# JoeyT1994/TensorNetworkQuantumSimulator.jl

Measured on AMD Instinct MI355X. Metric: two-site gates/sec at fixed chi (LxL TFIM Trotter layer), higher is better.
Workload: dtype c64 (ComplexF32; Gram/eigen steps in f64; the chi = 32 plane products as exact bf16 x 3 splits with f32 accumulation, TNQS_NO_BF16X3=1 for f32 matrix instructions)

## Files before the change

### include/tnqs_debug.h

```cpp
#ifndef TNQS_DEBUG_H
#define TNQS_DEBUG_H
#include <stdint.h>
#include "tnqs.h"
#ifdef __cplusplus
extern "C" {
#endif
int tnqs_dbg_jacobi(int dtype, int m, int n, void* A_inout, void* V_out, int* sweeps_out);
int tnqs_dbg_theta_svd_pre(int m, int n, int nq, void* A_inout, const void* Q, void* V_out, int* sweeps_out, int copies, int reps, double* ms_out, double* phase_us_out ,
                           int cap );
int tnqs_dbg_time_jacobi_f32(int m, int n, const void* A, int copies, int reps, double* ms_out, int* sweeps_out);
int tnqs_dbg_chol(int n, const void* G, void* L_out, void* W_out, int* fail_out, double tau);
int tnqs_dbg_fiber_gemm(int dtype, int D, int PA, int K, int PB, int Do, int No, const void* in, const void* X, void* out,
                        double* norm2_out, int use_mfma);
int tnqs_dbg_gram(int dtype, int D, int PA, int K, int PB, const void* X, const void* Y, void* out, int acc64, int use_mfma);
int tnqs_dbg_gram_fused(int PA, int K, int PB, const void* X, const void* Y, const void* M, void* out);
int tnqs_dbg_gauge_gram(int z, const int* chi, int bleg, const void* X, const void* M, void* out);
int tnqs_dbg_pair(int C0, int NMID, int NHI, const void* in, const void* Mx, const void* My, void* out);
int tnqs_dbg_pair_legs(int d, int z, const int* chi, int lx, int ly, const void* in, const void* Mx, const void* My, void* out);
int tnqs_dbg_pair_gram(int d, int z, const int* chi, int lx, int ly, const void* X, const void* Y, const void* M, void* out);
int tnqs_dbg_pair_gram2(int d, int z, const int* chi, int lx, int ly, const void* X, const void* Y, const void* Mx, const void* My, void* out_y, void* out_x);
int tnqs_dbg_bench_plane(int which, int nsites, int lx, int ly, int reps, double* ms);
#define TNQS_DBG_ROUTE_X3 1
#define TNQS_DBG_ROUTE_F32 2
#define TNQS_DBG_ROUTE_F64 3
#define TNQS_DBG_ROUTE_F64_SHARED 4
#define TNQS_DBG_ROUTE_HALF_LINES 5
#define TNQS_DBG_ROUTE_WHOLE_LINES 6
#define TNQS_DBG_ROUTE_SMALL_SCALAR 7
#define TNQS_DBG_ROUTE_SMALL_MFMA16 8
int tnqs_dbg_rowgemm(int D, int K, int nitems, const int* PA, const int* PB, const int* No, const void* in, const void* X, void* out, double* norm2_out,
                     int tpw, int* route_out);
int tnqs_dbg_gram_mfma(int nitems, const int* shape, const void* X, const void* Y, void* out, int nchunks, int* route_out);
int tnqs_dbg_pair16(int d, int nitems, const int* z, const int* chi, const int* lx, const int* ly, const void* in, const void* M, void* out, int spw, int* route_out);
int tnqs_dbg_pair_gram2x16(int d, int nitems, const int* z, const int* chi, const int* lx, const int* ly, const int* both, const void* X, const void* Y, const void* M,
                           void* out_y, void* out_x, int spw);
int tnqs_dbg_pair32(int d, int nitems, const int* z, const int* chi, const int* lx, const int* ly, const void* in, const void* M, void* out, int spw, int guard,
                    int* route_out, int* spw_out, int* wg_begin_out, int* nwg_out, int* total_wgs_out);
int tnqs_dbg_pair_gram32(int d, int nitems, const int* z, const int* chi, const int* lx, const int* ly, int form, const void* X, const void* Y, const void* M,
                         void* out_y, void* out_x, int spw, int guard, int* route_out, int* spw_out, int* wg_begin_out, int* nwg_out, int* total_wgs_out);
int tnqs_dbg_svd_tall(int nitems, const int* m, const int* n, void* A, int* chol_fail, int* polished, int* sweeps);
int tnqs_dbg_small_site(int nitems, const int* d, const int* z, const int* chi, const int* jo, const void* psi, const void* M, const int* present, int form,
                        const void* old_msg, const int* has_old, int normalize, void* out, void* new_msg, double* diff_out, int* route_out);
int tnqs_dbg_msg_finalize(int dtype, int nitems, const int* chi, const int* nchunks, const void* partials, const void* old_msg, const int* has_old, int normalize,
                          void* new_msg, double* diff_out);
int tnqs_dbg_default_sequence(tnqs_handle h, int* src, int* dst, int cap, int* n_out);
int tnqs_dbg_default_sequence_graph(int nv, int ne, const int32_t* esrc, const int32_t* edst, int* src, int* dst, int* level, int cap, int* n_out);
int tnqs_dbg_gate_schedule(int nv, int ne, const int32_t* esrc, const int32_t* edst, int ngates, const int32_t* nverts, const int32_t* verts, int update_cache,
                           int* step_of_gate, int* step_is_bp, int cap, int* nsteps_out);
int tnqs_dbg_fiber_plan(int use, int dtype, int use_mfma, int use_chi64, int nitems, const int* shape, int* launches_out, int cap, int* nlaunches_out, int* items_out);
int tnqs_dbg_loop_cgemm(int dtype, int opB, int nitems, const int* m, const int* n, const int* k, const void* A, const void* B, void* C, int guard);
int tnqs_dbg_loop_antiproject(int dtype, int nitems, const int* nr, const int* nc, void* T_inout, const void* f, const void* b);
int tnqs_dbg_loop_trace(int dtype, int nitems, const int* p, const int* q, const void* X, const void* Y, double* out_re_im);
int tnqs_dbg_loop_branch_gram(int dtype, int nitems, const int* dims, const int* order, const int* k, const void* A, const void* B, void* C, int guard);
int tnqs_dbg_msg_rescale(int dtype, int nitems, const int* chi, const void* me, const void* mer, const int* present, void* me_out, void* mer_out, int guard);
int tnqs_dbg_edge_scalar(int dtype, int nitems, const int* chi, const void* me, const void* mer, const int* present, double* out_re_im);
int tnqs_dbg_env_prepare(int dtype, int nitems, const int* n, const void* msg, const int* present, void* H_out, void* V_out, int guard);
int tnqs_dbg_env_finish(int dtype, int nitems, const int* n, const void* A, const void* V, const double* cutoff, void* msqrt_out, void* proj_out, int* flags_out, int guard);
int tnqs_dbg_symg_build(int dtype, int nitems, const int* n, const void* AX, const void* VX, const void* AY, const void* VY, double reg, void* rx, void* ry, void* irx, void* iry,
                        void* Ce, void* Ce0, int* flag_out, int guard);
int tnqs_dbg_symg_finish(int dtype, int nitems, const int* n, const void* USigma, const void* Vsvd, const void* irx, const void* iry, void* Xs, void* Xd, double* S, int guard);
int tnqs_dbg_diag(int dtype, int nitems, const int* chi, const double* S, void* out, int guard);
int tnqs_dbg_cscale(int dtype, int nitems, const int* len, const void* src, const double* re, const double* im, void* dst, int guard);
int tnqs_dbg_edge_rdm(int ptype , int nitems, const int* du, const int* dv, const int* chi,
                      const int* nchunks_u, const int* nchunks_v, const void* partial_u, const void* partial_v,
                      const double* scale_u, const double* scale_v, void* out, int guard);
int tnqs_dbg_edge_rdm_mixed(int ptype_u , int ptype_v, int nitems, const int* du, const int* dv, const int* chi,
                            const int* nchunks_u, const int* nchunks_v, const void* partial_u, const void* partial_v,
                            const double* scale_u, const double* scale_v, void* out, int guard);
int tnqs_dbg_path_apply(int ptype_in , int dtype , int nitems, const int* d, const int* chi_a, const int* chi_b,
                        const int* nchunks_in, const int* ksplit, const void* L_in, const void* T, const double* scale , void* L_out, int guard);
int tnqs_dbg_path_apply_plan(int nitems, const int* chi_a, const int* chi_b, const int* ksplit, int* ksplit_out, int* nrb_out);
int tnqs_dbg_rdm_paths_ws(tnqs_handle h, int npaths, const int32_t* path_len, const int32_t* path_verts, double* out,
                          int64_t workspace_bytes, int* nbatches_out);
int tnqs_dbg_rdm_edges_ws(tnqs_handle h, int n_edges, const int32_t* eu, const int32_t* ev, double* out,
                          int64_t workspace_bytes, int* nbatches_out);
int tnqs_dbg_bond_spectrum(int dtype, int nitems, const int* chi, const void* m1, const void* m2, const int* present, double* out, int* flags_out, int guard);
int tnqs_dbg_pending_scale(tnqs_handle h, int v, double* factor);
int tnqs_dbg_operator_sum(const void* gate, int d1, int d2, int* kappa_out, void* fa_out, void* fb_out);
int tnqs_dbg_gate_theta(int dtype, int nitems, const int* dims, const int* mode, const int* rk, const void* F1, const void* F2, const double* tau, const void* gate,
                        const int* maxdim, int lowrank_on, int stop_after, int* low_sizes_out, int* info, double* lam1, double* lam2, int* idx1, int* idx2,
                        void* theta, void* theta0, void* thetaV, void* lowA, void* lowB, void* lowG, void* lowL, void* lowQ, void* lowL2c, int* texp, int* lowfail, int guard);
int tnqs_dbg_gate_finish(int dtype, int nitems, const int* dims, const int* info_in, const int* texp, const void* theta, const void* thetaV, const double* lam1, const double* lam2,
                         const int* idx1, const int* idx2, const void* GW1, const void* GW2, const int* maxdim, const double* cutoff, const int* normalize, const int* chi_cap,
                         double* S, int* info_out, double* truncerr, void* X1, void* X2, int guard);
#define TNQS_DBG_ROUTE_SVD_PRE_LOWRANK 10
#define TNQS_DBG_ROUTE_SVD_PRE_THETA 11
#define TNQS_DBG_ROUTE_SVD_LDS 12
#define TNQS_DBG_ROUTE_SVD_GLOBAL 13
#define TNQS_DBG_ROUTE_SVD_TALL 14
int tnqs_dbg_theta_svd_stage(int dtype, int dyn, int nitems, const int* dims, const int* info, const int* K, const int* has_q, const void* Q, const int* rank_bounds, const int* cap,
                             int recover_form, void* theta, void* theta0, void* thetaV, int* sweeps_out, int* route_out, int guard);
int tnqs_dbg_qr2(int stage, int nitems, const int* n, const void* GW, const void* GV, const double* lam, const int* idx, const int* r, const void* A2, const void* V2, const double* tau,
                 void* X1, void* GVout, void* GWout, int* rk, int guard);
int tnqs_dbg_small_svd(int dtype, int nitems, const int* shape, const void* src, void* GA, void* GV, int guard);
#define TNQS_DBG_ROUTE_INNER_MFMA 9
int tnqs_dbg_inner_gram(int dtype, int nitems, const int* shape, const void* X, const void* Y, void* out, int max_chunks, int* nchunks_out, int guard, int* route_out);
int tnqs_dbg_inner_finalize(int dtype, int nitems, const int* rows, const int* cols, const int* nchunks, const void* partials, const void* old_msg, const int* has_old,
                            const int* normalize, void* new_msg, double* diff_out, double* sum_out, int guard);
int tnqs_dbg_inner_scalar(int dtype, int nitems, const int* rows, const int* cols, const void* m, const void* mr, const int* present, const double* rawsum, const int* has_rawsum,
                          const int* normalize, const double* scale_a, const double* scale_b, const int* has_scale, double* out_re_im, int guard);
int tnqs_dbg_site_prob(int dtype, int n, int d, const void* tabs, const void* psi, int nblocks, double* partial, int guard, int* nblocks_out);
int tnqs_dbg_site_draw(int nitems, const int* nblocks, const int* d, const double* partials, const double* neg_tol, const double* uniform, const int* use_counter,
                       const uint64_t* counter, const int* draw, double* p_out, int* x_out, double* px_out, int* status_out, int guard);
int tnqs_dbg_site_project(int dtype, int nout, int d, const void* psi, int x, int x_on_device, void* out, int guard);
int tnqs_dbg_site1(int nitems, const int* npairs, const void* in, const double* gates, int nbx, int normalize, void* out, double* partials, double* factors, int guard);
int tnqs_dbg_norm_factor(int nitems, const int* npart, const double* partials, double* factors, int guard);
int tnqs_dbg_scale(int dtype, int nitems, const int* len, const void* src, const double* factor, void* dst, int guard);
int tnqs_dbg_inner_bp_ws(tnqs_handle ket, tnqs_handle bra, const tnqs_bp_opts* opts, double* out_log_re_im, int* niter, double* final_diff, int64_t workspace_bytes, int* nbatches_out);
int tnqs_dbg_amp_leg_gemm(int dtype, int nitems, const int* shape, const void* T, const int32_t* x, const void* M, const int* has_m, void* R, int guard);
int tnqs_dbg_amp_absorb(int dtype, int nitems, const int* shape, const void* in, const void* m, const int* has_m, void* out, int guard);
int tnqs_dbg_amp_finalize(int dtype, int nitems, const int* chi, const int* nstr, const void* raw, const void* old_msg, const int* has_old, const int* normalize, const int* done,
                          void* new_msg, double* diff_out, double* sum_out, int guard);
int tnqs_dbg_amplitudes_bp_ws(tnqs_handle h, int nstrings, const int32_t* configs, const tnqs_bp_opts* opts, double* out_log_re_im, int32_t* niter, double* final_diff,
                              int32_t* flags, int64_t workspace_bytes, int* nbatches_out);
#define TNQS_DBG_ROUTE_FIBER_GENERIC 15
#define TNQS_DBG_ROUTE_FIBER_F64_PLAIN 16
#define TNQS_DBG_ROUTE_FIBER_F64_GENERAL 17
#define TNQS_DBG_ROUTE_GRAM_GENERIC 18
#define TNQS_DBG_ROUTE_GRAM_F64IN 19
int tnqs_dbg_fiber_pass_c128(int use, int use_mfma, int nitems, const int* shape, const int* want_norm, const void* in, const void* X, void* out, double* partials, int tpw,
                             int guard, int* route_out, int* inst_out, int* wg_begin_out, int* nwg_out);
int tnqs_dbg_gram_c128(int use_mfma, int nitems, const int* shape, const int* same, const void* X, const void* Y, void* out, int max_chunks, int* nchunks_out, int guard,
                       int* route_out);
int tnqs_dbg_gram_route(int dtype, int acc64, int has_m, int all_same, int all_f64in, int kkmax, int use_mfma, int use_chi64, int* route_out);
#ifdef __cplusplus
}
#endif
#endif
```

### tensornetworkquantumsimulator.jl_amd/csrc/debug_plane.cpp

```cpp
#include "debug_util.hpp"

using namespace tnqs;

extern "C" int tnqs_dbg_pair(int C0, int NMID, int NHI, const void* in, const void* Mx, const void* My, void* out) {
    return guard([&] {
        need_gpu();
        if (C0 % 16) throw Err(TNQS_ERR_INVALID, "dbg_pair: C0 % 16 != 0");
        size_t n = (size_t)C0 * 32 * NMID * 32 * NHI;
        DBuf dIn(n * 8), dOut(n * 8), dX(32 * 32 * 8), dY(32 * 32 * 8); DevItems<PairItem> dI(1);
        dIn.up(in, n * 8); dX.up(Mx, 32 * 32 * 8); dY.up(My, 32 * 32 * 8);
        HIPCHK(hipMemset(dOut.p, 0xff, n * 8));
        PairItem it{}; it.in = dIn.p; it.out = dOut.p; it.Mx = dX.p; it.My = dY.p;
        it.g.cstr = 2; it.g.sx = C0; it.g.sy = (long long)C0 * 32 * NMID; it.g.n0 = C0 / 16; it.g.t0 = 16; it.g.n1 = NMID; it.g.t1 = (long long)C0 * 32;
        it.g.n2 = NHI; it.g.t2 = (long long)C0 * 32 * NMID * 32;
        const int wgs = plan_pair(&it, 1, 3);
        dI.up(it);
        launch_mfma_pair(nullptr, dI.get(), 1, wgs);
        HIPCHK(hipDeviceSynchronize());
        dOut.down(out, n * 8);
    });
}
extern "C" int tnqs_dbg_pair_legs(int d, int z, const int* chi, int lx, int ly, const void* in, const void* Mx, const void* My, void* out) {
    return guard([&] {
        need_gpu();
// ... 209 lines not shown
        plane_items(d, nitems, z, chi, lx, ly, g, off);
        const bool wl = pair16_whole_lines(g[0]);
        for (int i = 0; i < nitems; ++i) if (pair16_whole_lines(g[i]) != wl) throw Err(TNQS_ERR_UNSUPPORTED, "dbg_pair16: one launch holds items of one kind");
        if (spw > 0 && spw % 4) throw Err(TNQS_ERR_INVALID, "dbg_pair16: spw must be a multiple of 4");
        const size_t n = off[nitems];
        DBuf dIn(n * 8), dOut(n * 8), dM((size_t)nitems * 512 * 8); DevItems<Pair16Item> dI(nitems);
        dIn.up(in, n * 8); dM.up(M, (size_t)nitems * 512 * 8);
        HIPCHK(hipMemset(dOut.p, 0xff, n * 8));
        std::vector<Pair16Item> items(nitems);
        for (int i = 0; i < nitems; ++i) {
            Pair16Item& it = items[i]; it.g = g[i]; it.in = (char*)dIn.p + off[i] * 8; it.out = (char*)dOut.p + off[i] * 8;
            it.Mx = (char*)dM.p + (size_t)i * 512 * 8; it.My = (char*)it.Mx + 256 * 8;
        }
        int wgs[2]; plan_pair16(items.data(), nitems, wgs, spw);
        dI.up(items);
        launch_mfma_pair16(nullptr, dI.get(), nitems, wgs[wl ? 1 : 0], wl);
        HIPCHK(hipDeviceSynchronize());
        dOut.down(out, n * 8);
        if (route) *route = wl ? TNQS_DBG_ROUTE_WHOLE_LINES : TNQS_DBG_ROUTE_HALF_LINES;
    });
}
extern "C" int tnqs_dbg_pair_gram2x16(int d, int nitems, const int* z, const int* chi, const int* lx, const int* ly, const int* both, const void* X, const void* Y, const void* M,
                                      void* out_y, void* out_x, int spw) {
    return guard([&] {
        need_gpu();
        std::vector<PlaneGeom> g; std::vector<size_t> off;
        plane_items(d, nitems, z, chi, lx, ly, g, off);
        if (!both) throw Err(TNQS_ERR_INVALID, "dbg_pair_gram2x16: bad arguments");
        if (spw > 0 && spw % pair_gram2x16_slices_at_a_time()) throw Err(TNQS_ERR_INVALID, "dbg_pair_gram2x16: spw must be a multiple of the slices a workgroup walks at a time");
        const size_t n = off[nitems];
        std::vector<PairGram2x16Item> items(nitems); std::vector<int> nwg(nitems); for (int i = 0; i < nitems; ++i) items[i].g = g[i];
        const int wgs = plan_pair_gram2x16(items.data(), nitems, nwg.data(), spw);
        DBuf dX(n * 8), dY(n * 8), dM((size_t)nitems * 512 * 8); DevItems<PairGram2x16Item> dI(nitems); DBuf dP((size_t)2 * wgs * 256 * 8), dO((size_t)2 * nitems * 256 * 8);
        DevItems<ReduceItem> dR(2 * (size_t)nitems);
        dX.up(X, n * 8); dY.up(Y, n * 8); dM.up(M, (size_t)nitems * 512 * 8);
        HIPCHK(hipMemset(dO.p, 0, (size_t)2 * nitems * 256 * 8));
        std::vector<ReduceItem> ri;
        for (int i = 0; i < nitems; ++i) {
            PairGram2x16Item& it = items[i];
            it.X = (char*)dX.p + off[i] * 8; it.Y = (char*)dY.p + off[i] * 8;
            it.Mx = (char*)dM.p + (size_t)i * 512 * 8; it.My = both[i] ? (const void*)((char*)it.Mx + 256 * 8) : nullptr;
            it.partial_y = (char*)dP.p + (size_t)it.wg_begin * 256 * 8;
            it.partial_x = both[i] ? (void*)((char*)dP.p + ((size_t)wgs + it.wg_begin) * 256 * 8) : nullptr;
            ri.push_back(ReduceItem{it.partial_y, (char*)dO.p + (size_t)i * 256 * 8, 256, nwg[i], 0, (int)ri.size() * 256});
            if (both[i]) ri.push_back(ReduceItem{it.partial_x, (char*)dO.p + ((size_t)nitems + i) * 256 * 8, 256, nwg[i], 0, (int)ri.size() * 256});
        }
        dI.up(items); dR.up(ri);
        launch_mfma_pair_gram2x16(nullptr, dI.get(), nitems, wgs);
        launch_reduce<float, float>(nullptr, dR.get(), (int)ri.size(), (int)ri.size() * 256);
        HIPCHK(hipDeviceSynchronize());
        dO.down(out_y, (size_t)nitems * 256 * 8);
        if (out_x) for (int i = 0; i < nitems; ++i) if (both[i]) HIPCHK(hipMemcpy((char*)out_x + (size_t)i * 256 * 8, (char*)dO.p + ((size_t)nitems + i) * 256 * 8, 256 * 8, hipMemcpyDeviceToHost));
    });
}

namespace {
void pair32_geoms(const char* who, int d, int nitems, const int* z, const int* chi, const int* lx, const int* ly, int spw, int guard_elems, std::vector<PairGeom>& g,
                  std::vector<size_t>& n) {
    if (nitems < 1 || !z || !chi || !lx || !ly || d < 1 || guard_elems < 0 || spw > (1 << 16)) throw Err(TNQS_ERR_INVALID, std::string(who) + ": bad arguments");
    g.resize(nitems); n.resize(nitems);
    int c = 0;
    for (int i = 0; i < nitems; ++i) {
        if (z[i] < 2 || z[i] > 8) throw Err(TNQS_ERR_INVALID, std::string(who) + ": 2 <= z <= 8");
        n[i] = d;
        for (int k = 0; k < z[i]; ++k) { if (chi[c + k] < 1 || chi[c + k] > 1024) throw Err(TNQS_ERR_INVALID, std::string(who) + ": 1 <= chi <= 1024"); n[i] *= chi[c + k]; }
        if (!pair_geometry(d, z[i], chi + c, lx[i], ly[i], g[i]) || (size_t)g[i].n0 * g[i].n1 * g[i].n2 * 16 * 1024 != n[i])
            throw Err(TNQS_ERR_UNSUPPORTED, std::string(who) + ": shape not covered by the chi = 32 plane kernels");
        c += z[i];
    }
}
template <class Item> void plan_report(const std::vector<Item>& items, int Item::*begin, int total, int* spw_out, int* wg_begin_out, int* nwg_out, int* total_wgs_out) {
    const int n = (int)items.size();
    if (spw_out) *spw_out = items[0].spw;
    for (int i = 0; i < n; ++i) {
        if (wg_begin_out) wg_begin_out[i] = items[i].*begin;
        if (nwg_out) nwg_out[i] = (i + 1 < n ? items[i + 1].*begin : total) - items[i].*begin;
    }
    if (total_wgs_out) *total_wgs_out = total;
}
}
extern "C" int tnqs_dbg_pair32(int d, int nitems, const int* z, const int* chi, const int* lx, const int* ly, const void* in, const void* M, void* out, int spw, int guard_elems,
                               int* route, int* spw_out, int* wg_begin_out, int* nwg_out, int* total_wgs_out) {
    return guard([&] {
        std::vector<PairGeom> g; std::vector<size_t> n;
        pair32_geoms("dbg_pair32", d, nitems, z, chi, lx, ly, spw, guard_elems, g, n);
        if (in && (!M || !out)) throw Err(TNQS_ERR_INVALID, "dbg_pair32: bad arguments");
        std::vector<PairItem> items(nitems);
        for (int i = 0; i < nitems; ++i) { items[i] = PairItem{}; items[i].g = g[i]; }
        const int wgs = plan_pair(items.data(), nitems, spw);
        plan_report(items, &PairItem::slice_begin, wgs, spw_out, wg_begin_out, nwg_out, total_wgs_out);
        if (route) *route = mfma_use_x3() ? TNQS_DBG_ROUTE_X3 : TNQS_DBG_ROUTE_F32;
        if (!in) return;
        need_gpu();
        Slots sIn, sM; Guarded gO((size_t)guard_elems * 8);
        for (int i = 0; i < nitems; ++i) { sIn.add(n[i] * 8); sM.add(2 * 1024 * 8); gO.add(n[i] * 8); }
        alloc_all(sIn, sM, gO); put_all(sIn, in); put_all(sM, M);
        for (int i = 0; i < nitems; ++i) { PairItem& it = items[i]; it.in = sIn.at(i); it.out = gO.at(i); it.Mx = sM.at(i); it.My = sM.at(i) + 1024 * 8; }
        DevItems<PairItem> dI(items);
        up_all(sIn, sM); gO.up(out);
        launch_mfma_pair(nullptr, dI.get(), nitems, wgs);
        HIPCHK(hipDeviceSynchronize());
        gO.down(out, "out");
    });
}
extern "C" int tnqs_dbg_pair_gram32(int d, int nitems, const int* z, const int* chi, const int* lx, const int* ly, int form, const void* X, const void* Y, const void* M,
                                    void* out_y, void* out_x, int spw, int guard_elems, int* route, int* spw_out, int* wg_begin_out, int* nwg_out, int* total_wgs_out) {
    return guard([&] {
        std::vector<PairGeom> g; std::vector<size_t> n;
        pair32_geoms("dbg_pair_gram32", d, nitems, z, chi, lx, ly, spw, guard_elems, g, n);
        if ((form != 0 && form != 1) || (X && (!Y || !M || !out_y || (form == 0 && !out_x)))) throw Err(TNQS_ERR_INVALID, "dbg_pair_gram32: bad arguments");
        const bool x3 = mfma_use_x3(), f32_single = form == 1 && !x3;
        std::vector<PairGram2Item> two(nitems); std::vector<PairGramItem> one(f32_single ? nitems : 0);
        std::vector<int> nwg(nitems); int wgs = 0;
        for (int i = 0; i < nitems; ++i) { two[i] = PairGram2Item{}; two[i].g = g[i]; if (f32_single) { one[i] = PairGramItem{}; one[i].g = g[i]; } }
        if (form == 0) wgs = plan_pair_gram2(two.data(), nitems, nwg.data(), spw);
        else if (x3) wgs = plan_x3_pair_gram1(two.data(), nitems, nwg.data(), spw);
        else wgs = plan_pair_gram(one.data(), nitems, nwg.data(), spw);
        if (f32_single) plan_report(one, &PairGramItem::wg_begin, wgs, spw_out, wg_begin_out, nwg_out, total_wgs_out);
        else plan_report(two, &PairGram2Item::wg_begin, wgs, spw_out, wg_begin_out, nwg_out, total_wgs_out);
        if (route) *route = x3 ? TNQS_DBG_ROUTE_X3 : TNQS_DBG_ROUTE_F32;
        if (!X) return;
        need_gpu();
        const size_t band = 256, pb = 1024 * 8;
        const int nmsg = form == 0 ? 2 : 1;
        Slots sX, sY, sM, sP(band); Guarded gOy((size_t)guard_elems * 8), gOx((size_t)guard_elems * 8);
        for (int i = 0; i < nitems; ++i) {
            sX.add(n[i] * 8); sY.add(n[i] * 8); sM.add(2 * pb); gOy.add(pb); gOx.add(pb);
            for (int m = 0; m < nmsg; ++m) sP.add((size_t)nwg[i] * pb);
        }
        alloc_all(sX, sY, sM, sP, gOy); put_all(sX, X); put_all(sY, Y); put_all(sM, M);
        if (form == 0) gOx.alloc();
        std::vector<ReduceItem> ri;
        for (int i = 0; i < nitems; ++i) {
            void* py = sP.at((size_t)nmsg * i); void* px = form == 0 ? sP.at((size_t)nmsg * i + 1) : nullptr;
            if (f32_single) { PairGramItem& it = one[i]; it.X = sX.at(i); it.Y = sY.at(i); it.M = sM.at(i); it.partial = py; }
            else { PairGram2Item& it = two[i]; it.X = sX.at(i); it.Y = sY.at(i); it.Mx = sM.at(i); it.My = form == 0 ? sM.at(i) + pb : nullptr; it.partial_y = py; it.partial_x = px; }
            ri.push_back(ReduceItem{py, gOy.at(i), 1024, nwg[i], 0, (int)ri.size() * 1024});
            if (form == 0) ri.push_back(ReduceItem{px, gOx.at(i), 1024, nwg[i], 0, (int)ri.size() * 1024});
        }
        DevItems<PairGram2Item> dTwo(two); DevItems<PairGramItem> dOne(one); DevItems<ReduceItem> dR(ri);
        up_all(sX, sY, sM, sP); gOy.up(out_y); if (form == 0) gOx.up(out_x);
        if (form == 0) launch_mfma_pair_gram2(nullptr, dTwo.get(), nitems, wgs);
        else if (x3) launch_x3_pair_gram1(nullptr, dTwo.get(), nitems, wgs);
        else launch_mfma_pair_gram(nullptr, dOne.get(), nitems, wgs);
        launch_reduce<float, float>(nullptr, dR.get(), (int)ri.size(), (int)ri.size() * 1024);
        HIPCHK(hipDeviceSynchronize());
        sP.down("the pair-Gram partials");
        auto untouched = [&](size_t b0, size_t b1) { for (size_t b = b0; b < b1; ++b) if (sP.host[b] != (char)0xff) throw Err(TNQS_ERR_INVALID, "dbg: a kernel wrote outside an item of the pair-Gram partials"); };
        untouched(0, band);
        for (size_t k = 0; k < sP.off.size(); ++k) untouched(sP.off[k] + sP.len[k], sP.off[k] + sP.len[k] + band);
        gOy.down(out_y, "out_y"); if (form == 0) gOx.down(out_x, "out_x");
    });
}
```

### tensornetworkquantumsimulator.jl_amd/csrc/engine_bp.cpp

```cpp
#include "engine_internal.hpp"
#include "launch_util.hpp"

namespace tnqs {

static int fused_leg(const State* s, const SD& sd, int jo) {
    if (s->dtype != TNQS_C64 || !use_mfma() || sd.d != 2 || sd.z < 2) return -1;
    int r = (jo == 0) ? 1 : 0;
    if (sd.chi[r] != 32 || sd.chi[jo] > 32 || sd.chi[jo] < 8) return -1;
    return r;
}

static double default_tol(const State* s) { return s->dtype == TNQS_C64 ? 1e-5 : 1e-8; }
static bool small_site_on() { static const bool v = !envflag("TNQS_NO_SMALL_SITE_BP"); return v; }

struct SharedT { Buf site, ma, mb, T; int la = -1, lb = -1; };

typedef std::vector<std::pair<int, Buf>> LegBufs;
struct ProdEntry { Buf site; LegBufs legs; Buf prod; long long next_use = 0; };
static void drop_legs(LegBufs& want, const LegBufs& have) {
    LegBufs rest; for (auto& w : want) { bool in = false; for (auto& b : have) in = in || b.first == w.first; if (!in) rest.push_back(w); }
    want.swap(rest);
}
struct SweepClock { int level = 0, iter = 1, maxiter = 1; };
struct ProdCache {
// ... 153 lines not shown
        }
        const double* st_tot = readback<double>(s, d_sum->p, 1);
        sync(s);
        const double tot = *st_tot;
        settle(s, true);
        avg = tot / (double)nseq;
        if (avg <= tol) { converged = true; niter = iter; return BpVerdict::Converged; }
        return BpVerdict::Continue;
    }
    void commit(int* niter_out, double* diff_out) {
        sync(s);
        settle(s, true);
        s->msg = cur;
        if (iters_before == 0) s->stats.n_bp_updates += 1;
        if (compute_error && !converged) s->stats.bp_not_converged += 1;
        s->stats.last_bp_diff = avg;
        if (niter_out) *niter_out = niter;
        if (diff_out) *diff_out = compute_error ? avg : -1.0;
    }
};

template <class T> struct BpLevelBatch {
    enum class Route { Small,
                       Pair32Single,
                       Pair32Double,
                       Plane16Double,
                       Plane16Single,
                       GenericFused,
                       GenericPlain };
    struct Msg { int t, src, jo; Route route; const void* fused = nullptr; int item = -1; };
    struct Prefix { Buf site; std::vector<std::pair<int, const void*>> legs; Buf prod, bra; bool has_bra = false; };
    struct Pend { int msg, jo, r; };
    struct Continued { LegBufs base, absorbed; };

    BpUpdate<T>& u; State* const s; const Graph& g; const BPPlan& plan; const std::vector<int>& lev; const size_t start, esz; size_t end;
    std::vector<Msg> msgs; std::vector<Chain> chains;
    std::unordered_map<size_t, Continued> continued;
    std::vector<PairItem> sh_pair; std::vector<PairGramItem> pair32_items;
    std::vector<PairGram2Item> sh_dbl; std::vector<std::pair<int, int>> sh_dbl_msg;
    std::vector<SmallMsgItem> small_items; std::vector<int> small_msg; int small_max = 0;
    std::unordered_map<long long, Pend> pend;
    double sh_pair_slices = 0, sh_dbl_slices = 0;
    std::unordered_map<int, Prefix> prefix;
    std::vector<Buf> hits_alive;
    std::vector<PairGram2x16Item> g16; std::vector<std::pair<int, int>> g16_msg;
    std::vector<int> g16_single;
    hipStream_t main_stream = nullptr, side_stream = nullptr; bool split_level = false;
    std::vector<size_t> slot;
    std::vector<GramJob> jobs;

    BpLevelBatch(BpUpdate<T>& up, const std::vector<int>& level, size_t first)
        : u(up), s(up.s), g(up.g), plan(up.plan), lev(level), start(first), esz(up.esz), end(first) {}
    void take() {
        const size_t budget = bp_ws_budget(); size_t used = 0;
        while (end < lev.size()) {
            const size_t need = 2 * site_dims(s, g.src_of(plan.seq[lev[end]])).n * esz;
            if (end > start && used + need > budget) break;
            used += need; ++end;
        }
    }
    static bool generic(Route r) { return r == Route::GenericFused || r == Route::GenericPlain; }

    bool continue_from_remembered(Chain& c, LegBufs& want, LegBufs& base) {
        ProdEntry hit;
        if (!u.pcache.find(c.v, s->site[c.v], want, hit)) return false;
        base = hit.legs; c.src = hit.prod->p; hits_alive.push_back(hit.prod);
        drop_legs(want, base);
        return true;
    }

    void shared_prefixes() {
        if (plan.in_place) return;
        std::unordered_map<int, std::vector<int>> outl;
        auto generic_site = [&](int src, int jo) { const SD sd = site_dims(s, src); return (u.tshare.empty() || sd.z != 4 || u.partner[src][jo] < 0) && !u.small_site(sd); };
        for (size_t q = start; q < end; ++q) {
            const int de = plan.seq[lev[q]], src = g.src_of(de), jo = g.leg(src, g.dst_of(de));
            if (s->owns(src) && generic_site(src, jo)) outl[src].push_back(jo);
        }
        std::vector<Chain> pch; std::vector<int> psrc, pside; std::vector<LegBufs> pbase, pabs;
        auto start_product = [&](int src, LegBufs w, int side) {
            Prefix& pf = prefix[src];
            Chain cp; cp.v = src; cp.src = s->site[src]->p; cp.sd = site_dims(s, src);
            LegBufs base;
            if (u.cache_on) {
                cp.ordered = true;
                if (continue_from_remembered(cp, w, base)) (side ? pf.bra : pf.prod) = hits_alive.back();
            }
            for (auto& x : w) cp.steps.push_back({x.first, x.second->p});
            if (cp.steps.empty()) return;
            pch.push_back(std::move(cp)); psrc.push_back(src); pside.push_back(side); pbase.push_back(std::move(base)); pabs.push_back(std::move(w));
        };
        for (size_t q = start; q < end; ++q) {
            const int t = lev[q], src = g.src_of(plan.seq[t]);
            auto ol = outl.find(src);
            if (ol == outl.end() || ol->second.size() < 2 || prefix.count(src)) continue;
            const SD sd = site_dims(s, src);
            Prefix pf; pf.site = s->site[src];
            LegBufs want;
            for (int j = 0; j < sd.z; ++j) {
                if (std::find(ol->second.begin(), ol->second.end(), j) != ol->second.end()) continue;
                const Buf& mb = u.incoming(src, j, t);
                if (!mb) continue;
                want.push_back({j, mb});
            }
            if (want.empty()) continue;
            if (u.cache_on || u.bra_on) u.by_stability(want, src, t);
            const size_t nket = (u.bra_on && want.size() >= 4) ? (want.size() + 1) / 2 : want.size();
            for (size_t i = 0; i < want.size(); ++i) pf.legs.push_back({want[i].first, want[i].second->p});
            prefix[src] = pf;
            start_product(src, LegBufs(want.begin(), want.begin() + (std::ptrdiff_t)nket), 0);
            if (nket < want.size()) { prefix[src].has_bra = true; start_product(src, LegBufs(want.begin() + (std::ptrdiff_t)nket, want.end()), 1); }
        }
        if (pch.empty()) return;
        run_chains<T>(s, pch, TNQS_PROF_BP_MODEPROD, TNQS_PROF_BP_PAIR);
        for (size_t i = 0; i < pch.size(); ++i) {
            Prefix& pf = prefix[psrc[i]];
            for (int k = 0; k < 2; ++k) if (pch[i].tmp[k] && pch[i].tmp[k]->p == pch[i].result) (pside[i] ? pf.bra : pf.prod) = pch[i].tmp[k];
            if (u.cache_on) u.remember(pch[i], pf.site, pbase[i], pabs[i]);
        }
    }

    void route_messages() {
        for (size_t q = start; q < end; ++q) {
            const int t = lev[q], de = plan.seq[t], src = g.src_of(de);
            if (!s->owns(src)) continue;
            Chain c; c.v = src; c.src = s->site[src]->p; c.sd = site_dims(s, src);
            Msg m{}; m.t = t; m.src = src; m.jo = g.leg(src, g.dst_of(de));
            if (u.small_site(c.sd)) route_small(m, c);
            else if (!route_pair32(m, c)) route_generic(m, c);
            msgs.push_back(m); chains.push_back(std::move(c));
        }
    }
    void route_small(Msg& m, const Chain& c) {
        SmallMsgItem si{}; si.psi = c.src; si.d = c.sd.d; si.z = c.sd.z; si.jo = m.jo;
        for (int j = 0; j < c.sd.z; ++j) {
            si.chi[j] = c.sd.chi[j]; si.M[j] = nullptr;
            if (j == m.jo) continue;
            const Buf& mb = u.incoming(m.src, j, m.t);
            if (mb) si.M[j] = mb->p;
        }
        si.mfma = bp_small_site_mfma_form(c.sd.z, c.sd.chi.data(), c.sd.n) ? 1 : 0;
        small_items.push_back(si); small_msg.push_back((int)msgs.size()); small_max = std::max(small_max, (int)c.sd.n);
        m.route = Route::Small;
    }
    bool route_pair32(Msg& m, const Chain& c) {
        const int src = m.src, jo = m.jo;
        if (u.tshare.empty() || c.sd.z != 4 || u.partner[src][jo] < 0) return false;
        const int r = u.partner[src][jo];
        int pa = -1, pb = -1;
        for (int j = 0; j < 4; ++j) if (j != jo && j != r) { if (pa < 0) pa = j; else pb = j; }
        const Buf& ma = u.incoming(src, pa, m.t); const Buf& mb = u.incoming(src, pb, m.t); const Buf& mr = u.incoming(src, r, m.t);
        PairGramItem gi{}; PairItem pi{};
        if (!(ma && mb && mr && pair_geometry(c.sd.d, c.sd.z, c.sd.chi.data(), pa, pb, pi.g) && pair_geometry(c.sd.d, c.sd.z, c.sd.chi.data(), r, jo, gi.g))) return false;
        const int slot = std::min(pa, pb) < std::min(r, jo) ? 0 : 1;
        SharedT& sh = u.tshare[src][slot];
        if (!(sh.T && sh.site == s->site[src] && sh.ma == ma && sh.mb == mb && sh.la == pa && sh.lb == pb)) {
            sh.site = s->site[src]; sh.ma = ma; sh.mb = mb; sh.la = pa; sh.lb = pb;
            sh.T = dalloc(s, c.sd.n * esz);
            pi.in = c.src; pi.out = sh.T->p; pi.Mx = ma->p; pi.My = mb->p;
            sh_pair.push_back(pi); sh_pair_slices += (double)c.sd.n / 16384.0;
        }
        gi.X = sh.T->p; gi.Y = c.src; gi.M = mr->p;
        m.item = (int)pair32_items.size(); pair32_items.push_back(gi);
        const long long key = ((long long)src << 1) | slot;
        auto pit = pend.find(key);
        if (pit != pend.end() && pit->second.jo == r && pit->second.r == jo && pair32_items[msgs[pit->second.msg].item].X == gi.X) {
            Msg& mf = msgs[pit->second.msg]; const PairGramItem& first = pair32_items[mf.item];
            PairGram2Item d2{}; d2.X = first.X; d2.Y = first.Y; d2.Mx = first.M; d2.My = gi.M; d2.g = first.g;
            sh_dbl.push_back(d2); sh_dbl_msg.push_back({pit->second.msg, (int)msgs.size()});
            sh_dbl_slices += (double)c.sd.n / 8192.0;
            mf.route = m.route = Route::Pair32Double;
            pend.erase(pit);
        } else {
            pend[key] = Pend{(int)msgs.size(), jo, r};
            m.route = Route::Pair32Single;
        }
        return true;
    }
    void route_generic(Msg& m, Chain& c) {
        const int src = m.src, jo = m.jo, t = m.t;
        const int fr = fused_leg(s, c.sd, jo);
        std::vector<char> done(c.sd.z, 0);
        {
            auto pf = prefix.find(src);
            if (pf != prefix.end() && pf->second.prod && (!pf->second.has_bra || pf->second.bra) && pf->second.site == s->site[src]) {
                bool same = true;
                for (auto& lm : pf->second.legs) { if (lm.first == jo) { same = false; break; } const Buf& mb = u.incoming(src, lm.first, t); if (!mb || mb->p != lm.second) { same = false; break; } }
                if (same) { c.y = pf->second.has_bra ? pf->second.bra->p : c.src; c.src = pf->second.prod->p; for (auto& lm : pf->second.legs) done[lm.first] = 1; }
            }
        }
        LegBufs want, base;
        for (int j = 0; j < c.sd.z; ++j) {
            if (j == jo || done[j]) continue;
            const Buf& mb = u.incoming(src, j, t);
            if (!mb) continue;
            want.push_back({j, mb});
        }
        const bool from_prefix = c.y != nullptr;
        if (u.cache_on && !from_prefix) {
            u.by_stability(want, src, t); c.ordered = true;
            const void* psi = c.src;
            if (continue_from_remembered(c, want, base)) c.y = psi;
        }
        for (auto& w : want) {
            if (w.first == fr) m.fused = w.second->p;
            else c.steps.push_back({w.first, w.second->p});
        }
        if (u.cache_on && !from_prefix) continued[msgs.size()] = Continued{std::move(base), std::move(want)};
        m.route = m.fused ? Route::GenericFused : Route::GenericPlain;
    }

    void pair_up_planes16() {
        if (!(std::is_same<T, float>::value && use_mfma() && use_pair())) return;
        std::unordered_map<int, std::vector<int>> by_src;
        for (size_t ci = 0; ci < chains.size(); ++ci)
            if (chains[ci].y && chains[ci].steps.size() == 1 && !msgs[ci].fused && chains[ci].sd.n >= (size_t)(1u << 14)) by_src[chains[ci].v].push_back((int)ci);
        for (auto& kv : by_src) {
            if (kv.second.size() != 2) continue;
            const int ci = kv.second[0], cj = kv.second[1];
            Chain& a = chains[ci]; Chain& b = chains[cj];
            const int ly = msgs[ci].jo, lx = msgs[cj].jo;
            if (a.src != b.src || a.y != b.y || a.steps[0].first != lx || b.steps[0].first != ly) continue;
            PairGram2x16Item it{};
            if (!plane_geometry(a.sd.d, a.sd.z, a.sd.chi.data(), lx, ly, 16, it.g)) continue;
            it.X = a.src; it.Y = a.y; it.Mx = a.steps[0].second; it.My = b.steps[0].second;
            g16.push_back(it); g16_msg.push_back({ci, cj});
            a.steps.clear(); b.steps.clear();
            msgs[ci].route = msgs[cj].route = Route::Plane16Double;
        }
        for (size_t ci = 0; ci < chains.size(); ++ci) {
            Chain& c = chains[ci];
            if (!generic(msgs[ci].route)) continue;
            auto ct = continued.find(ci);
            if ((c.y && (ct == continued.end() || ct->second.base.empty())) || msgs[ci].fused || c.steps.empty() || (c.steps.size() & 1) == 0 || c.sd.n < (size_t)(1u << 14)) continue;
            const int ly = msgs[ci].jo, lx = c.steps.back().first;
            PairGram2x16Item it{};
            if (!plane_geometry(c.sd.d, c.sd.z, c.sd.chi.data(), lx, ly, 16, it.g)) continue;
            bool all16 = true; for (auto& st : c.steps) all16 = all16 && c.sd.chi[st.first] == 16;
            if (!all16) continue;
            it.Y = c.y ? c.y : c.src; it.Mx = c.steps.back().second; it.My = nullptr; it.X = nullptr;
            c.steps.pop_back();
            g16_single.push_back((int)g16.size());
            g16.push_back(it); g16_msg.push_back({(int)ci, -1});
            msgs[ci].route = Route::Plane16Single;
        }
    }

    struct SplitGuard { State* s; hipStream_t m; bool on; ~SplitGuard() { s->stream = m; if (on) s->pool->set_defer(false); } };
    void on_side(bool side) { if (split_level) { s->stream = side ? side_stream : main_stream; s->prof->chain = false; } }
    void fork() {
        main_stream = s->stream;
        bool has_other = false;
        for (const Msg& m : msgs) has_other = has_other || m.route == Route::Small || generic(m.route);
        split_level = (!sh_pair.empty() || !sh_dbl.empty()) && has_other && g16.empty();
        if (!split_level) return;
        side_stream = aux_stream_of(s);
        HIPCHK(hipEventRecord(s->ev_fork, main_stream)); HIPCHK(hipStreamWaitEvent(side_stream, s->ev_fork, 0));
        s->pool->set_defer(true);
    }
    void join() { if (split_level) { HIPCHK(hipEventRecord(s->ev_join, side_stream)); HIPCHK(hipStreamWaitEvent(main_stream, s->ev_join, 0)); } }

    void launch_products() {
        if (!sh_pair.empty()) {
            const int wgs = plan_pair(sh_pair.data(), (int)sh_pair.size());
            const PairItem* d = upload(s, sh_pair);
            ProfScope ps(s, TNQS_PROF_BP_PAIR, 2.0 * sh_pair_slices * 16384.0 * esz, 2 * 8.0 * sh_pair_slices * 16384.0 * 32);
            launch_mfma_pair(s->stream, d, (int)sh_pair.size(), wgs);
        }
        on_side(true);
        run_chains<T>(s, chains, TNQS_PROF_BP_MODEPROD, TNQS_PROF_BP_PAIR);
        on_side(false);
        if (u.cache_on) for (auto& kv : continued) if (!chains[kv.first].trail.empty()) u.remember(chains[kv.first], s->site[chains[kv.first].v], kv.second.base, kv.second.absorbed);
        for (size_t i = 0; i < chains.size(); ++i) {
            GramJob j{}; j.X = chains[i].result; j.Y = chains[i].y ? chains[i].y : chains[i].src; j.sd = chains[i].sd; j.leg = msgs[i].jo; j.keep_site = false;
            j.M = msgs[i].fused;
            jobs.push_back(j);
        }
    }
    void launch_small_sites() {
        if (small_items.empty()) return;
        size_t slab_bytes = 0;
        for (size_t q = 0; q < small_items.size(); ++q) { const int co = small_items[q].chi[small_items[q].jo]; slab_bytes += round256((size_t)co * co * esz); }
        Buf slab = dalloc(s, slab_bytes); size_t off = 0;
        for (size_t q = 0; q < small_items.size(); ++q) {
            GramJob& j = jobs[small_msg[q]];
            const int co = small_items[q].chi[small_items[q].jo];
            j.nchunks = 1; j.KK = co; j.partial = sub_buffer(slab, off, (size_t)co * co * esz); off += round256((size_t)co * co * esz);
            small_items[q].out = j.partial->p;
        }
        if (!s->sharded() && !plan.in_place) {
            size_t nb_bytes = 0;
            for (size_t q = 0; q < small_items.size(); ++q) if (small_items[q].mfma) nb_bytes += round256((size_t)256 * esz);
            if (nb_bytes) {
                Buf nslab = dalloc(s, nb_bytes); size_t noff = 0;
                for (size_t q = 0; q < small_items.size(); ++q) {
                    SmallMsgItem& si = small_items[q]; if (!si.mfma) continue;
                    GramJob& j = jobs[small_msg[q]];
                    const int t = msgs[small_msg[q]].t; const int de = plan.seq[t];
                    j.final_msg = sub_buffer(nslab, noff, (size_t)256 * esz); noff += round256((size_t)256 * esz);
                    si.new_msg = j.final_msg->p; si.old_msg = u.cur[de] ? u.cur[de]->p : nullptr;
                    si.diff_out = reinterpret_cast<double*>(u.d_diffs->p) + t; si.normalize = u.normalize;
                }
            }
        }
        on_side(true);
        const SmallMsgItem* d = upload_small(s, small_items);
        { ProfScope ps(s, TNQS_PROF_BP_FUSED, 0, 0); launch_bp_small_site(s->stream, d, (int)small_items.size(), small_max); }
        on_side(false);
    }
    template <class Item, class PlanFn, class LaunchFn>
    void launch_pair32_singles(std::vector<Item>& items, void* Item::*partial, const std::vector<int>& of_msg, double slices, PlanFn plan_fn, LaunchFn launch_fn) {
        std::vector<int> nwg(items.size()); const int wgs = plan_fn(items.data(), (int)items.size(), nwg.data(), 0);
        for (size_t q = 0; q < items.size(); ++q) {
            GramJob& j = jobs[of_msg[q]];
            j.nchunks = nwg[q]; j.KK = 32; j.partial = dalloc(s, (size_t)j.nchunks * 1024 * esz);
            items[q].*partial = j.partial->p;
        }
        const Item* d = upload(s, items);
        ProfScope ps(s, TNQS_PROF_BP_PAIRGRAM, 2.0 * slices * 16384.0 * esz, 2 * 8.0 * slices * 16384.0 * 32);
        launch_fn(s->stream, d, (int)items.size(), wgs);
    }
    void launch_plane_grams() {
        if (!sh_dbl.empty()) {
            std::vector<int> nwg(sh_dbl.size()); const int wgs = plan_pair_gram2(sh_dbl.data(), (int)sh_dbl.size(), nwg.data());
            for (size_t q = 0; q < sh_dbl.size(); ++q) {
                PairGram2Item& it = sh_dbl[q]; GramJob& jy = jobs[sh_dbl_msg[q].first]; GramJob& jx = jobs[sh_dbl_msg[q].second];
                jy.nchunks = jx.nchunks = nwg[q]; jy.KK = jx.KK = 32;
                jy.partial = dalloc(s, (size_t)jy.nchunks * 1024 * esz); jx.partial = dalloc(s, (size_t)jx.nchunks * 1024 * esz);
                it.partial_y = jy.partial->p; it.partial_x = jx.partial->p;
            }
            const PairGram2Item* d = upload(s, sh_dbl);
            ProfScope ps(s, TNQS_PROF_BP_PAIRGRAM, 2.0 * sh_dbl_slices * 8192.0 * esz, 4 * 8.0 * sh_dbl_slices * 8192.0 * 32);
            launch_mfma_pair_gram2(s->stream, d, (int)sh_dbl.size(), wgs);
        }
        for (int q : g16_single) g16[q].X = chains[g16_msg[q].first].result;
        if (!g16.empty()) {
            std::vector<int> nwgs(g16.size()); const int wgs = plan_pair_gram2x16(g16.data(), (int)g16.size(), nwgs.data()); double by = 0, fl = 0;
            for (size_t q = 0; q < g16.size(); ++q) {
                PairGram2x16Item& it = g16[q]; GramJob& jy = jobs[g16_msg[q].first]; const int nwg = nwgs[q];
                jy.nchunks = nwg; jy.KK = 16; jy.partial = dalloc(s, (size_t)nwg * 256 * esz); it.partial_y = jy.partial->p;
                if (g16_msg[q].second >= 0) {
                    GramJob& jx = jobs[g16_msg[q].second];
                    jx.nchunks = nwg; jx.KK = 16; jx.partial = dalloc(s, (size_t)nwg * 256 * esz); it.partial_x = jx.partial->p;
                } else it.partial_x = nullptr;
                by += 2.0 * jy.sd.n * esz; fl += (g16_msg[q].second >= 0 ? 4 : 2) * 8.0 * jy.sd.n * 16;
            }
            const PairGram2x16Item* d = upload(s, g16);
            ProfScope ps(s, TNQS_PROF_BP_PAIRGRAM, by, fl);
            launch_mfma_pair_gram2x16(s->stream, d, (int)g16.size(), wgs);
        }
        std::vector<PairGramItem> singles; std::vector<int> single_msg; double slices = 0;
        for (size_t i = 0; i < msgs.size(); ++i) if (msgs[i].route == Route::Pair32Single) {
            singles.push_back(pair32_items[msgs[i].item]); single_msg.push_back((int)i); slices += (double)chains[i].sd.n / 16384.0;
        }
        if (singles.empty()) return;
        if (mfma_use_x3()) {
            std::vector<PairGram2Item> one(singles.size());
            for (size_t q = 0; q < singles.size(); ++q) { const PairGramItem& a = singles[q]; one[q].X = a.X; one[q].Y = a.Y; one[q].Mx = a.M; one[q].g = a.g; }
            launch_pair32_singles(one, &PairGram2Item::partial_y, single_msg, slices, plan_x3_pair_gram1, launch_x3_pair_gram1);
        } else launch_pair32_singles(singles, &PairGramItem::partial, single_msg, slices, plan_pair_gram, launch_mfma_pair_gram);
    }
    void launch_generic_grams() {
        std::vector<GramJob> jf, jp; std::vector<size_t> idf, idp;
        for (size_t i = 0; i < jobs.size(); ++i) {
            if (msgs[i].route == Route::GenericFused) { jf.push_back(jobs[i]); idf.push_back(i); }
            else if (msgs[i].route == Route::GenericPlain) { jp.push_back(jobs[i]); idp.push_back(i); }
        }
        on_side(true);
        run_grams<T, T>(s, jf, TNQS_PROF_BP_FUSED);
        run_grams<T, T>(s, jp, TNQS_PROF_BP_GRAM);
        join();
        on_side(false);
        for (size_t q = 0; q < jf.size(); ++q) jobs[idf[q]] = jf[q];
        for (size_t q = 0; q < jp.size(); ++q) jobs[idp[q]] = jp[q];
    }

    MsgFinalItem final_item(int t, const void* partial, int nchunks) {
        const int de = plan.seq[t], c = s->chi[de / 2];
        Buf nb = dalloc(s, (size_t)c * c * esz);
        MsgFinalItem f{}; f.partial = partial; f.nchunks = nchunks; f.chi = c;
        const Buf& oldb = plan.in_place && u.fresh[de] ? u.fresh[de] : u.cur[de];
        f.old_msg = oldb ? oldb->p : nullptr; f.new_msg = nb->p;
        f.diff_out = reinterpret_cast<double*>(u.d_diffs->p) + t; f.normalize = u.normalize;
        u.fresh[de] = nb;
        return f;
    }
    void finalize() {
        std::vector<MsgFinalItem> fin;
        if (!s->sharded()) {
            for (size_t i = 0; i < jobs.size(); ++i) {
                if (jobs[i].final_msg) u.fresh[plan.seq[msgs[i].t]] = jobs[i].final_msg;
                else fin.push_back(final_item(msgs[i].t, jobs[i].partial->p, jobs[i].nchunks));
            }
        } else {
            const size_t stride = exchange_raw_messages();
            const char* base = reinterpret_cast<const char*>(s->exch);
            for (size_t q = start; q < end; ++q) fin.push_back(final_item(lev[q], base + (size_t)s->owner[g.src_of(plan.seq[lev[q]])] * stride + slot[q - start], 1));
        }
        if (!fin.empty()) {
            const MsgFinalItem* d = upload_small(s, fin);
            ProfScope ps(s, TNQS_PROF_SMALL, 0, 0);
            launch_msg_finalize<T>(s->stream, d, (int)fin.size());
        }
    }
    size_t exchange_raw_messages() {
        slot.assign(end - start, 0); std::vector<size_t> rank_bytes(s->nranks, 0);
        for (size_t q = start; q < end; ++q) {
            const int de = plan.seq[lev[q]], r = s->owner[g.src_of(de)];
            slot[q - start] = rank_bytes[r];
            rank_bytes[r] += round256((size_t)s->chi[de / 2] * s->chi[de / 2] * esz);
        }
        size_t stride = 0; for (size_t b : rank_bytes) stride = std::max(stride, b);
        check_exchange(s, stride);
        char* base = reinterpret_cast<char*>(s->exch);
        std::vector<ReduceItem> ri; int elems = 0; size_t oi = 0;
        for (size_t q = start; q < end; ++q) {
            const int de = plan.seq[lev[q]];
            if (!s->owns(g.src_of(de))) continue;
            const int n2 = s->chi[de / 2] * s->chi[de / 2];
            ri.push_back(ReduceItem{jobs[oi].partial->p, base + (size_t)s->rank * stride + slot[q - start], n2, jobs[oi].nchunks, 0, elems});
            elems += n2; ++oi;
        }
        if (!ri.empty()) { const ReduceItem* dr = upload(s, ri); launch_reduce<T, T>(s->stream, dr, (int)ri.size(), elems); }
        exchange(s, stride);
        return stride;
    }

    void run() {
        HostTimer ht_prep(0);
        take();
        shared_prefixes();
        route_messages();
        pair_up_planes16();
        ht_prep.stop();
        HostTimer ht_launch(1);
        fork();
        SplitGuard split_guard{s, main_stream, split_level};
        launch_products();
        launch_small_sites();
        launch_plane_grams();
        launch_generic_grams();
        ht_launch.stop();
        HostTimer ht_fin(2);
        finalize();
    }
};

template <class T> void BpUpdate<T>::sweep(int iter) {
    fresh.assign(2 * (size_t)g.ne, nullptr);
    at.iter = iter; at.level = -1;
    for (auto& lev : plan.levels) {
        ++at.level;
        for (size_t start = 0; start < lev.size();) {
            BpLevelBatch<T> b(*this, lev, start);
            b.run();
            start = b.end;
        }
    }
    for (size_t t = 0; t < nseq; ++t) if (fresh[plan.seq[t]]) cur[plan.seq[t]] = fresh[plan.seq[t]];
    s->stats.n_bp_sweeps += 1;
}

template <class T> void bp_update_t(State* s, const tnqs_bp_opts* o, int* niter_out, double* diff_out, bool optimistic, int iters_before) {
    HIPCHK(hipSetDevice(s->device));
    const std::shared_ptr<const BPPlan> plan = plan_for(*s->g, o);
    if (!(o ? o->normalize : 1)) materialize_scale_all(s);
    if (plan->seq.empty()) { if (niter_out) *niter_out = 0; if (diff_out) *diff_out = 0; return; }
    PhaseScope phase_scope(s, TNQS_PROF_PHASE_BP_UPDATE); phase_scope.count = 0;
    BpUpdate<T> u(s, *plan, o, optimistic, iters_before);
    for (int iter = 1 + iters_before; iter <= u.at.maxiter; ++iter) {
        phase_scope.count += 1;
        u.sweep(iter);
        const BpVerdict v = u.verdict(iter);
        if (v == BpVerdict::Deferred) return;
        if (v == BpVerdict::Converged) break;
    }
    u.commit(niter_out, diff_out);
}

void bp_update(State* s, const tnqs_bp_opts* o, int* niter, double* diff) {
    if (s->dtype == TNQS_C64) bp_update_t<float>(s, o, niter, diff); else bp_update_t<double>(s, o, niter, diff);
}

template void bp_update_t<float>(State*, const tnqs_bp_opts*, int*, double*, bool, int);
template void bp_update_t<double>(State*, const tnqs_bp_opts*, int*, double*, bool, int);

}
```

### tensornetworkquantumsimulator.jl_amd/csrc/engine_internal.hpp

```cpp
#pragma once
#include "engine.hpp"
#include "kernels.hpp"
#include <algorithm>
#include <array>
#include <chrono>
#include <climits>
#include <cmath>
#include <complex>
#include <cstdio>
#include <cstdlib>
#include <cstring>
#include <functional>
#include <limits>
#include <memory>
#include <mutex>
#include <numeric>
#include <set>
#include <type_traits>
#include <unordered_map>

namespace tnqs {

#define HIPCHK(x) hipchk((x), #x)

inline bool envflag(const char* name) { const char* e = std::getenv(name); return e && e[0] == '1'; }
#define TNQS_SWITCH(fn, expr) inline bool fn() { static const bool v = (expr); return v; }
TNQS_SWITCH(use_mfma, !envflag("TNQS_NO_MFMA"))
TNQS_SWITCH(use_pair, !envflag("TNQS_NO_PAIR"))
TNQS_SWITCH(use_bra_products, !envflag("TNQS_NO_BRA_PRODUCTS"))
TNQS_SWITCH(use_prodcache, !envflag("TNQS_NO_PRODCACHE"))
TNQS_SWITCH(use_chol, !envflag("TNQS_NO_CHOL"))
TNQS_SWITCH(use_qr2, !envflag("TNQS_NO_QR2"))
TNQS_SWITCH(use_lowrank, !envflag("TNQS_NO_LOWRANK"))
TNQS_SWITCH(use_precond_svd, !envflag("TNQS_NO_PRECOND_SVD"))
TNQS_SWITCH(use_small_svd, !envflag("TNQS_NO_SMALLSVD"))
TNQS_SWITCH(defer_site1, !envflag("TNQS_NO_DEFER_1SITE"))
TNQS_SWITCH(use_chi64, !envflag("TNQS_NO_CHI64"))
TNQS_SWITCH(speculation_on, !envflag("TNQS_NO_SPECULATION"))
#undef TNQS_SWITCH
inline size_t bp_cache_budget() { static const size_t v = [] { const char* e = std::getenv("TNQS_BP_CACHE_MB"); return (e ? (size_t)std::atoll(e) : (size_t)49152) << 20; }(); return v; }
inline size_t bp_ws_budget() { static const size_t v = [] { const char* e = std::getenv("TNQS_BP_WS_MB"); return (e ? (size_t)std::atoll(e) : (size_t)24576) << 20; }(); return v; }
inline size_t jacobi_lds(size_t bytes) { static const bool g = envflag("TNQS_JACOBI_GLOBAL"); return (g || bytes > 160 * 1024 - 2048) ? 0 : bytes; }
inline int mmax_of(const std::vector<JacobiItem>& ji) { int m = 1; for (auto& j : ji) m = std::max(m, std::max(j.m, j.n)); return m; }

struct HostTimer {
    static double acc[16]; static long cnt[16];
    int k; std::chrono::steady_clock::time_point t0; bool on;
    explicit HostTimer(int kk) : k(kk), t0(std::chrono::steady_clock::now()), on(true) {}
    void stop() { if (on) { static std::mutex mu; std::lock_guard<std::mutex> lk(mu); acc[k] += std::chrono::duration<double, std::milli>(std::chrono::steady_clock::now() - t0).count(); cnt[k]++; on = false; } }
    ~HostTimer() { stop(); }
};

void sync(State* s);
hipStream_t aux_stream_of(State* s);
void recycle_arena(HostArena ar);
HostArena acquire_arena();
inline void drain_for_arena_reuse(State* s) {
    HIPCHK(hipStreamSynchronize(s->stream));
    if (s->aux_stream && s->aux_stream != s->stream) HIPCHK(hipStreamSynchronize(s->aux_stream));
}
template <class X> const X* readback(State* s, const void* dsrc, size_t count) {
    const size_t bytes = count * sizeof(X);
    HostArena& ar = s->arena;
    if (!ar.base) ar = acquire_arena();
    const size_t aligned = (std::max<size_t>(bytes, 1) + 255) & ~size_t(255);
    if (aligned > ar.cap) throw Err(TNQS_ERR_UNSUPPORTED, "read-back too large for the staging arena");
    if (ar.off + aligned > ar.cap) { drain_for_arena_reuse(s); ar.off = 0; }
    char* h = ar.base + ar.off; ar.off += aligned;
    if (bytes) HIPCHK(hipMemcpyAsync(h, dsrc, bytes, hipMemcpyDeviceToHost, s->stream));
    return reinterpret_cast<const X*>(h);
}
inline void reserve_readback(State* s, size_t bytes) {
    HostArena& ar = s->arena;
    if (!ar.base) ar = acquire_arena();
    if (bytes > ar.cap) throw Err(TNQS_ERR_UNSUPPORTED, "read-backs of one batch too large for the staging arena");
    if (ar.off + bytes > ar.cap) { drain_for_arena_reuse(s); ar.off = 0; }
}
inline void soft_sync(State* s) { s->keep_mark = s->keepalive.size(); }
inline void drained(State* s) {
    s->prof->chain = false;
    s->arena.off = 0;
    if (s->keep_mark) { s->keepalive.erase(s->keepalive.begin(), s->keepalive.begin() + (std::ptrdiff_t)std::min(s->keep_mark, s->keepalive.size())); s->keep_mark = 0; }
}
void materialize_scale(State* s, const std::vector<int>& verts);
void materialize_scale_all(State* s);
void materialize_pending(State* s, const std::vector<int>& verts);
void materialize_pending_all(State* s);
inline Buf dalloc(State* s, size_t bytes) {
    auto b = std::make_shared<DevBuf>();
    b->pool = s->pool; b->bytes = bytes;
    b->p = s->pool->alloc(bytes ? bytes : 1, &b->rounded);
    return b;
}
template <class Item> const Item* upload(State* s, const std::vector<Item>& v) {
    if (v.empty()) return nullptr;
    size_t bytes = v.size() * sizeof(Item);
    HostArena& ar = s->arena;
    if (!ar.base) ar = acquire_arena();
    size_t aligned = (bytes + 255) & ~size_t(255);
    if (aligned > ar.cap) throw Err(TNQS_ERR_UNSUPPORTED, "descriptor batch too large");
    if (ar.off + aligned > ar.cap) { drain_for_arena_reuse(s); ar.off = 0; s->prof->chain = false; }
    char* h = ar.base + ar.off; ar.off += aligned;
    std::memcpy(h, v.data(), bytes);
    Buf b = dalloc(s, bytes);
    HIPCHK(hipMemcpyAsync(b->p, h, bytes, hipMemcpyHostToDevice, s->stream));
    s->keepalive.push_back(b);
    return reinterpret_cast<const Item*>(b->p);
}

inline const void* upload_small_bytes(State* s, const void* p, size_t bytes) {
    HostArena& ar = s->arena;
    if (!ar.base) ar = acquire_arena();
    const size_t aligned = (bytes + 255) & ~size_t(255);
    if (aligned > ar.cap) throw Err(TNQS_ERR_UNSUPPORTED, "descriptor batch too large");
    if (ar.off + aligned > ar.cap) { drain_for_arena_reuse(s); ar.off = 0; s->prof->chain = false; }
    char* h = ar.base + ar.off; ar.off += aligned;
    std::memcpy(h, p, bytes);
    return h;
}
template <class Item> const Item* upload_small(State* s, const std::vector<Item>& v) {
    return v.empty() ? nullptr : static_cast<const Item*>(upload_small_bytes(s, v.data(), v.size() * sizeof(Item)));
}

struct ProfScope {
    State* s; int cls; hipEvent_t a = nullptr, b = nullptr; bool own_a = true;
    ProfScope(State* st, int c, double bytes, double flops) : s(st), cls(c) {
        Prof& P = *s->prof;
        if (!P.on) return;
        P.cls[c].bytes += bytes; P.cls[c].flops += flops; P.cls[c].launches += 1;
        auto get = [&]() { hipEvent_t e; if (!P.ev_free.empty()) { e = P.ev_free.back(); P.ev_free.pop_back(); } else HIPCHK(hipEventCreate(&e)); return e; };
        if (P.chain && P.last_b && P.last_stream == s->stream) { a = P.last_b; own_a = false; }
        else { a = get(); own_a = true; HIPCHK(hipEventRecord(a, s->stream)); }
        b = get();
    }
    ~ProfScope() {
        if (!a) return;
        Prof& P = *s->prof;
        (void)hipEventRecord(b, s->stream);
        P.pending.push_back({cls, a, b, own_a});
        P.last_b = b; P.chain = true; P.last_stream = s->stream;
    }
};

struct PhaseScope {
    State* s; int cls; hipEvent_t a = nullptr, b = nullptr; long count = 1;
    PhaseScope(State* st, int c) : s(st), cls(c) {
        Prof& P = *s->prof;
        if (!P.on) return;
        auto get = [&]() { hipEvent_t e; if (!P.ev_free.empty()) { e = P.ev_free.back(); P.ev_free.pop_back(); } else HIPCHK(hipEventCreate(&e)); return e; };
        a = get(); b = get();
        HIPCHK(hipEventRecord(a, s->stream));
    }
    ~PhaseScope() {
        if (!a) return;
        Prof& P = *s->prof;
        (void)hipEventRecord(b, s->stream);
        P.cls[cls].launches += count;
        P.pending.push_back({cls, a, b, true});
    }
};

struct ChiVec {
    int inl[8]; int n = 0; std::vector<int> big;
    void push_back(int c) { if (n < 8 && big.empty()) inl[n++] = c; else { if (big.empty()) big.assign(inl, inl + n); big.push_back(c); ++n; } }
    int* data() { return big.empty() ? inl : big.data(); }
    const int* data() const { return big.empty() ? inl : big.data(); }
    int& operator[](size_t i) { return data()[i]; }
    const int& operator[](size_t i) const { return data()[i]; }
    size_t size() const { return (size_t)n; }
    bool empty() const { return n == 0; }
    const int* begin() const { return data(); }
    const int* end() const { return data() + n; }
};
struct SD {
    int z = 0, d = 1; ChiVec chi; size_t n = 1;
    size_t pre(int j) const { size_t p = d; for (int i = 0; i < j; ++i) p *= chi[i]; return p; }
    size_t post(int j) const { size_t p = 1; for (int i = j + 1; i < z; ++i) p *= chi[i]; return p; }
};
inline SD site_dims(const State* s, int v) {
    SD r; const Graph& g = *s->g;
    r.z = (int)g.nbr[v].size(); r.d = s->d[v]; r.n = r.d;
    for (int j = 0; j < r.z; ++j) { int c = s->chi[g.nbr_e[v][j]]; r.chi.push_back(c); r.n *= c; }
    return r;
// ... 150 lines not shown
```

### tensornetworkquantumsimulator.jl_amd/csrc/kernels.hpp

```cpp
#pragma once
#include <algorithm>
#include <cstdlib>
#include <hip/hip_runtime_api.h>
#include <cstddef>
#include <cstdint>
#include <vector>

namespace tnqs {

struct FiberItem {
    const void* in; void* out; const void* X;
    int D, PA, K, PB;
    int Do, No;
    int TA, TB, nta, ntb;
    int tile_begin;
    int tpw;
    int want_norm;
};

struct GramItem {
    const void* X; const void* Y; void* partial;
    int D, PA, K, PB;
    int TA, TB, nta, ntb;
    int chunk_begin, nchunks, tiles_per_chunk;
// ... 122 lines not shown
[[noreturn]] void throw_unsupported(const char* what);
inline int pick_TR(size_t KK, size_t esz, int copies) {
    for (int tr : {64, 32, 16, 8, 4}) if (KK * tr * esz * copies <= 64 * 1024) return tr;
    throw_unsupported("bond dimension too large for the fiber-tile kernels (d*chi*16*elemsize must fit 64 KiB of LDS)");
}
inline void tile_params(size_t PA, size_t PB, int TR, int& TA, int& TB, int& nta, int& ntb) {
    TA = (int)std::min<size_t>(PA, TR); TB = std::max(1, TR / TA); TB = (int)std::min<size_t>(TB, PB);
    nta = (int)((PA + TA - 1) / TA); ntb = (int)((PB + TB - 1) / TB);
}

template <class T> void launch_fiber_gemm(hipStream_t s, const FiberItem* d_items, int nitems, int total_tiles,
                                          int TR, int KKmax, double* d_norm_partials);
inline int plan_fiber_gemm(FiberItem* it, int n, int TR, int tpw, int* nwg = nullptr) {
    for (int i = 0; i < n; ++i) tile_params(it[i].PA, it[i].PB, TR, it[i].TA, it[i].TB, it[i].nta, it[i].ntb);
    return lay_out(it, n, &FiberItem::tile_begin, nwg, [&](FiberItem& f) { f.tpw = tpw; return (f.nta * f.ntb + tpw - 1) / tpw; });
}
enum class FiberRoute { Generic, Mfma, RowGemm, F64 };
enum class FiberUse { Chain, Epilogue, Plain };
struct FiberRules {
    bool f32 = true, use_mfma = true, use_chi64 = true;
    int rg_D = 0, rg_cap = 0, rg_tpw = 0;
    bool matrix = false;
    bool general = false;
    int kk_min = 8, mfma_tpw = 0, f64_tpw = 0;
    int kk_floor = 1;
};
FiberRules fiber_rules(FiberUse use, bool f32, bool use_mfma, bool use_chi64);
struct FiberLaunch {
    FiberRoute route; int D, K;
    int TR, tpw, KKmax, NNmax, wgs; bool general;
    std::vector<FiberItem> items; std::vector<int> index, nwg;
};
std::vector<FiberLaunch> plan_fiber_pass(const FiberItem* items, int n, const FiberRules& r, size_t esz);
template <class T> void launch_fiber_route(hipStream_t s, const FiberLaunch& L, const FiberItem* d_items, double* d_norm_partials);
template <class T, class Acc> void launch_gram(hipStream_t s, const GramItem* d_items, int nitems, int total_chunks,
                                               int TR, int KKmax);
enum class GramRoute { Generic, Mfma32, Mfma64, Fused32, F64x64, F64x128, F64In, Gauge64, Gauge32 };
GramRoute gram_route(bool f32, bool acc64, bool has_M, bool all_same, bool all_f64in, size_t KKmax, bool use_mfma, bool use_chi64);
int gram_tile_rows(GramRoute r, size_t KKmax, size_t esz);
int plan_gram(GramItem* it, int n, GramRoute r, bool f32_acc64, int max_chunks, int* npart);
template <class T, class Acc> void launch_gram_route(hipStream_t s, GramRoute r, const GramItem* d_items, int nitems, int total_chunks, int TR, int KKmax,
                                                     bool all_full = false);
template <class Acc, class Out> void launch_reduce(hipStream_t s, const ReduceItem* d_items, int nitems, int total_elems);
template <class T> void launch_msg_finalize(hipStream_t s, const MsgFinalItem* d_items, int nitems);
struct RecoverItem { const void* A0; const void* A; void* V; int m; int n; int nu; const int* dyn; int dm, dn; int pre;  };
inline size_t jacobi_lds_bytes(int m, int n, bool withV, size_t esz) { return ((size_t)(m + 2) * n + (withV ? (size_t)(n + 2) * n : 0)) * esz; }
template <class T> void launch_jacobi(hipStream_t s, const JacobiItem* d_items, int nitems, int max_sweeps, size_t lds_bytes, int mmax, int ncols = 0);
inline bool theta_svd_pre_covers(int m, int n) { return n >= 2 && n <= 64 && m >= n && m <= 128; }
inline size_t theta_svd_pre_lds_bytes(int m, int n) { return ((((size_t)(m + 2) * n * 8) + 15) & ~(size_t)15) + (size_t)(n + 1) * n * 16; }
void launch_theta_svd_pre(hipStream_t s, const JacobiItem* d_items, int nitems, int max_sweeps, int mmax, int nmax);
struct SmallSvdItem { const void* src; void* M; void* GA; void* GV; int d, low, chi_b, hi; };
template <class T> void launch_small_svd_prepare(hipStream_t s, const SmallSvdItem* d_items, int nitems);
void launch_small_svd_finish(hipStream_t s, const SmallSvdItem* d_items, int nitems);
__host__ __device__ inline double rank_tau(bool f32_state, int n) { return f32_state ? 1e-12 : 4.0 * (double)n * 2.220446049250313e-16; }
struct CholItem { const void* G; void* L; void* Winv; int n; int* fail; double tau; double shift; };
struct TallSvdItem { const void* A; void* G; const void* L; void* R0; void* Rrot; int m, n; };
struct SmallGemmItem { const void* A; const void* B; void* C; int m, n, k; };
struct CopyItem { const void* src; void* dst; size_t n16; };
bool rowgemm_covers(const FiberItem& it);
void rowgemm_tiles(FiberItem& it);
int plan_rowgemm(FiberItem* it, int n, int cap, int* nwg = nullptr, int tpw = 0);
void launch_mfma_rowgemm(hipStream_t s, const FiberItem* d_items, int nitems, int total_wgs, int D, int K, double* d_norm_partials);
bool launch_x3_gram64(hipStream_t s, const GramItem* d_items, int nitems, int total_chunks, int KKmax);
void launch_x3_rowgemm64(hipStream_t s, const FiberItem* d_items, int nitems, int total_wgs, int D, double* d_norm_partials);
void launch_tall_gram(hipStream_t s, const TallSvdItem* d_items, int nitems, int nmax);
void launch_tall_rt(hipStream_t s, const TallSvdItem* d_items, int nitems);
void launch_tall_w(hipStream_t s, const TallSvdItem* d_items, int nitems, int nmax);
void launch_tall_mj(hipStream_t s, const SmallGemmItem* d_items, int nitems);
void launch_copy_items(hipStream_t s, const CopyItem* d_items, int nitems);
void launch_chol(hipStream_t s, const CholItem* d_items, int nitems, int nmax);
void launch_chol_packed(hipStream_t s, const CholItem* d_items, int nitems, int nmax);
template <class T> void launch_recover_v(hipStream_t s, const RecoverItem* d_items, int nitems, int nmax);
void launch_recover_v_mfma(hipStream_t s, const RecoverItem* d_items, int nitems, int nmax);
template <class T> void launch_env_prepare(hipStream_t s, const EnvItem* d_items, int nitems);
template <class T> void launch_env_finish(hipStream_t s, const EnvFinishItem* d_items, int nitems);
template <class T> void launch_gate_theta(hipStream_t s, const GateItem* d_items, int nitems);
template <class T> void launch_gate_theta_mm(hipStream_t s, const GateItem* d_items, int nitems);
template <class T> void launch_gate_finish(hipStream_t s, const GateItem* d_items, int nitems);
template <class T> void launch_diag(hipStream_t s, const DiagItem* d_items, int nitems);
template <class T> void launch_scale(hipStream_t s, const ScaleItem* d_items, int nitems);
void launch_norm_factor(hipStream_t s, const NormFactorItem* d_items, int nitems);
template <class T> void launch_permute(hipStream_t s, const PermItem& item);
template <class T> void launch_identity(hipStream_t s, void* out, int n);
template <class T> void launch_random_fill(hipStream_t s, void* out, size_t n, unsigned long long seed, double scale, bool real_only);
void launch_sum_doubles(hipStream_t s, const double* in, int n, double* out);
int plan_site_prob(size_t n, int d);
template <class T> void launch_site_prob_partial(hipStream_t s, const void* tabs, const void* psi, size_t n, int d, int nblocks, double* d_partial);
void launch_site_draw(hipStream_t s, const double* d_partial, int nblocks, int d, double neg_tol, const double* d_uniform, unsigned long long seed,
                      unsigned long long sample, unsigned long long step, bool draw, double* d_p, int* d_x, double* d_px, int* d_status);
template <class T> void launch_site_project(hipStream_t s, const void* psi, void* out, size_t nout, int d, const int* d_x, int x_host);
struct LoopGemmItem { const void* A; const void* B; void* C; int m, n, k, opB; int I0, J0; long long si0, si1, sj0, sj1;
                      int tile_begin, ntm, ntn; };
int plan_loop_cgemm(LoopGemmItem* it, int n);
template <class T> void launch_loop_cgemm(hipStream_t s, const LoopGemmItem* d_items, int nitems, int total_tiles);
struct BranchGramItem { const void* A; const void* B; void* C; int m, n, k; int R0, R1, C0, C1; long long sr[3], sc[3];
                        int tile_begin, ntm, ntn; };
int plan_loop_branch_gram(BranchGramItem* it, int n);
template <class T> void launch_loop_branch_gram(hipStream_t s, const BranchGramItem* d_items, int nitems, int total_tiles);
constexpr int kLoopDotMaxWgs = 1024;
struct LoopDotItem { const void* X; const void* Y; long long n; double* partial; double* out; int wg_begin, nwg; };
int plan_loop_dot(LoopDotItem* it, int n);
template <class T> void launch_loop_dot(hipStream_t s, const LoopDotItem* d_items, int nitems, int total_wgs);
struct LoopProjItem { void* T; const void* f; const void* b; int nr, nc; int wg_begin; };
int plan_loop_antiproject(LoopProjItem* it, int n);
template <class T> void launch_loop_antiproject(hipStream_t s, const LoopProjItem* d_items, int nitems, int total_wgs);
struct LoopTraceItem { const void* X; const void* Y; int p, q; double* partial; double* out; int wg_begin, nwg; };
int plan_loop_trace(LoopTraceItem* it, int n);
template <class T> void launch_loop_trace(hipStream_t s, const LoopTraceItem* d_items, int nitems, int total_wgs);
struct EdgeRdmItem { const void* partial_u; const void* partial_v; int nchunks_u, nchunks_v; int du, dv, chi; const double* scale_u; const double* scale_v; void* out; };
constexpr int kEdgeRdmLds = 64 * 1024;
__host__ __device__ inline int edge_rdm_block(int du, int dv, int chi) {
    const long long acc = 64ll * du * dv * du * dv, per = 16ll * ((long long)du * du + (long long)dv * dv) * chi;
    if (acc >= kEdgeRdmLds) return 0;
    const long long nb = (kEdgeRdmLds - acc) / per;
    return (int)(nb < chi ? nb : chi);
}
template <class P> void launch_edge_rdm(hipStream_t s, const EdgeRdmItem* d_items, int nitems);
template <class Pu, class Pv> void launch_edge_rdm_mixed(hipStream_t s, const EdgeRdmItem* d_items, int nitems);
struct PathApplyItem { const void* L_in; const void* T; void* L_out; const double* scale; int d, chi_a, chi_b, nchunks_in, ksplit; int wg_begin, nrb; };
constexpr int kPathApplyCols = 64;
constexpr int kPathApplyMaxSplit = 16;
constexpr int kPathApplyTargetWgs = 256;
int plan_path_apply(PathApplyItem* it, int n);
template <class P, class T> void launch_path_apply(hipStream_t s, const PathApplyItem* d_items, int nitems, int total_wgs);
struct InnerGramItem { const void* X; const void* Y; void* partial; int PA, Ka, Kb, PB; int chunk_begin, nchunks, blocks_per_chunk; };
inline bool inner_gram_covers(int Ka, int Kb) { return Ka >= 1 && Ka <= 64 && Kb >= 1 && Kb <= 64; }
int plan_inner_gram(InnerGramItem* it, int n, size_t esz, int max_chunks, int* npart);
template <class T> void launch_inner_gram(hipStream_t s, const InnerGramItem* d_items, int nitems, int total_chunks);
struct InnerFinalItem { const void* partial; int nchunks, rows, cols; const void* old_msg; void* new_msg; double* diff_out; double* sum_out; int normalize; };
template <class T> void launch_inner_finalize(hipStream_t s, const InnerFinalItem* d_items, int nitems);
struct InnerScalarItem { const void* m; const void* mr; int rows, cols; const double* rawsum; int normalize; const double* scale_a; const double* scale_b; double* out; };
template <class T> void launch_inner_scalar(hipStream_t s, const InnerScalarItem* d_items, int nitems);
struct AmpGemmItem { const void* T; const void* M; const int* idx; void* R; int d, PA, K, PB, ncols; int tile_begin, ntr, ntc; };
inline bool amp_covers(int K) { return K >= 1 && K <= 64; }
int plan_amp_gemm(AmpGemmItem* it, int n);
template <class T> void launch_amp_leg_gemm(hipStream_t s, const AmpGemmItem* d_items, int nitems, int total_tiles);
struct AmpAbsorbItem { const void* in; const void* m; void* out; int PA, K, PB, nstr; int wg_begin; };
int plan_amp_absorb(AmpAbsorbItem* it, int n);
template <class T> void launch_amp_absorb(hipStream_t s, const AmpAbsorbItem* d_items, int nitems, int total_wgs);
struct AmpFinalItem { const void* raw; const void* old_msg; void* new_msg; const int* done; double* diff_out; double* sum_out; int chi, nstr, normalize; int wg_begin; };
int plan_amp_finalize(AmpFinalItem* it, int n);
template <class T> void launch_amp_finalize(hipStream_t s, const AmpFinalItem* d_items, int nitems, int total_wgs);
void launch_amp_sweep_end(hipStream_t s, const double* diffs, int nseq, int nstrings, int iter, double tol, int* done, int* niter, double* fdiff);
struct AmpScalarItem { const void* m; const void* mr; const double* rawsum; const double* scale; const void* site; int chi, normalize, vertex; };
template <class T> void launch_amp_scalar(hipStream_t s, const AmpScalarItem* d_items, int nv, int ne, const int* cfg, int ld, int nstrings, double* out, int* flags);
void launch_site1_c64(hipStream_t s, const Site1Item* d_items, int nitems, int nbx, double* d_norm_partials);

struct PairGeom { long long cstr, sx, sy, t0, t1, t2; int n0, n1, n2; };
struct PairItem {
    const void* in; void* out; const void* Mx; const void* My;
    PairGeom g;
    int slice_begin;
    int spw;
};
struct PairGramItem {
    const void* X; const void* Y; const void* M; void* partial;
    PairGeom g;
    int wg_begin;
    int spw;
};

struct PlaneGeom { long long cstr, sx, sy, t0, t1, t2, t3; int n0, n1, n2, n3; int nslices() const { return n0 * n1 * n2 * n3; } };
inline bool plane_geometry(int d, int z, const int* chi, int lx, int ly, int DIM, PlaneGeom& g) {
    if (lx == ly || lx < 0 || ly < 0 || lx >= z || ly >= z || chi[lx] != DIM || chi[ly] != DIM) return false;
    auto pre = [&](int j) { long long p = d; for (int i = 0; i < j; ++i) p *= chi[i]; return p; };
    const int p = lx < ly ? lx : ly, q = lx < ly ? ly : lx;
    g.sx = pre(lx); g.sy = pre(ly);
    g.n1 = g.n2 = g.n3 = 1; g.t1 = g.t2 = g.t3 = 0;
    if (pre(p) % 16 == 0) {
        g.cstr = 2; g.n0 = (int)(pre(p) / 16); g.t0 = 16;
        g.n1 = (int)(pre(q) / (pre(p) * DIM)); g.t1 = pre(p) * DIM;
        long long post = 1; for (int i = q + 1; i < z; ++i) post *= chi[i];
        g.n2 = (int)post; g.t2 = pre(q) * DIM;
        return true;
    }
    if (pre(p) != 2) return false;
    int a = -1;
    for (int i = 0; i < z; ++i) if (i != p && i != q && chi[i] % 8 == 0) { a = i; break; }
    if (a < 0) return false;
    g.cstr = pre(a); g.n0 = chi[a] / 8; g.t0 = 8 * pre(a);
    int k = 0;
    for (int i = 0; i < z; ++i) {
        if (i == p || i == q || i == a) continue;
        if (k == 0) { g.n1 = chi[i]; g.t1 = pre(i); } else if (k == 1) { g.n2 = chi[i]; g.t2 = pre(i); } else if (k == 2) { g.n3 = chi[i]; g.t3 = pre(i); } else return false;
        ++k;
    }
    return true;
}
inline bool pair_geometry(int d, int z, const int* chi, int lx, int ly, PairGeom& g) {
    PlaneGeom p;
    if (!plane_geometry(d, z, chi, lx, ly, 32, p) || p.t3 != 0) return false;
    g = PairGeom{p.cstr, p.sx, p.sy, p.t0, p.t1, p.t2, p.n0, p.n1, p.n2};
    return true;
}
struct Pair16Item {
    const void* in; void* out; const void* Mx; const void* My;
    PlaneGeom g;
    int wg_begin;
    int spw;
};
struct PairGram2x16Item { const void* X; const void* Y; const void* Mx; const void* My; void* partial_y; void* partial_x; PlaneGeom g; int wg_begin; int spw; };
bool pair16_whole_lines(const PlaneGeom& g);
void plan_pair16(Pair16Item* it, int n, int wgs[2], int spw = 0);
void launch_mfma_pair16(hipStream_t s, const Pair16Item* d_items, int nitems, int total_wgs, bool whole_lines);
int pair_gram2x16_slices_at_a_time();
int plan_pair_gram2x16(PairGram2x16Item* it, int n, int* nwg = nullptr, int spw = 0);
void launch_mfma_pair_gram2x16(hipStream_t s, const PairGram2x16Item* d_items, int nitems, int total_wgs);

int mfma_fiber_tile_rows(int KK, int NN);
void launch_mfma_fiber_gemm(hipStream_t s, const FiberItem* d_items, int nitems, int total_tiles, int KKmax, int NNmax,
                            double* d_norm_partials);
bool launch_mfma_gram32(hipStream_t s, const GramItem* d_items, int nitems, int total_chunks, int KKmax);
bool launch_mfma_gram64(hipStream_t s, const GramItem* d_items, int nitems, int total_chunks, int KKmax);
void launch_mfma_gram32_fused(hipStream_t s, const GramItem* d_items, int nitems, int total_chunks);
bool launch_mfma_gram64_f64(hipStream_t s, const GramItem* d_items, int nitems, int total_chunks, int KKmax, bool all_kk64 = false);
bool fiber_gemm_f64_covers(const FiberItem& it);
int plan_fiber_gemm_f64(FiberItem* it, int n, int* nwg = nullptr, int tpw = 0);
void fiber_gemm_f64_inst(int Kmax, int Nmax, int* nblk, int* ks);
void launch_mfma_fiber_gemm_f64(hipStream_t s, const FiberItem* d_items, int nitems, int total_wgs, int Kmax, int Nmax, double* d_norm_partials, bool general);
bool gram_f64in_covers(int D, int K);
void launch_mfma_gram_f64in(hipStream_t s, const GramItem* d_items, int nitems, int total_chunks);
bool gauge_gram64_covers(int d, int z, const int* chi, int bleg, int rleg);
bool gauge_gram32_covers(int d, int z, const int* chi, int bleg, int rleg);
int gauge_gram32_units(int z, const int* chi, int bleg);
void launch_mfma_gauge_gram32(hipStream_t s, const GramItem* d_items, int nitems, int total_chunks);
void launch_mfma_gauge_gram64(hipStream_t s, const GramItem* d_items, int nitems, int total_chunks);
bool launch_mfma_gram128_f64(hipStream_t s, const GramItem* d_items, int nitems, int total_chunks, int KKmax, bool all_kk128 = false);
int plan_pair(PairItem* it, int n, int spw = 0);
void launch_mfma_pair(hipStream_t s, const PairItem* d_items, int nitems, int total_wgs);
void launch_x3_pair(hipStream_t s, const PairItem* d_items, int nitems, int total_wgs);
struct PairGram2Item { const void* X; const void* Y; const void* Mx; const void* My; void* partial_y; void* partial_x; PairGeom g; int wg_begin; int spw; };
int plan_pair_gram2(PairGram2Item* it, int n, int* nwg = nullptr, int spw = 0);
void launch_mfma_pair_gram2(hipStream_t s, const PairGram2Item* d_items, int nitems, int total_wgs);
void launch_x3_pair_gram2(hipStream_t s, const PairGram2Item* d_items, int nitems, int total_wgs);
int plan_x3_pair_gram1(PairGram2Item* it, int n, int* nwg = nullptr, int spw = 0);
void launch_x3_pair_gram1(hipStream_t s, const PairGram2Item* d_items, int nitems, int total_wgs);
int plan_pair_gram(PairGramItem* it, int n, int* nwg = nullptr, int spw = 0);
void launch_mfma_pair_gram(hipStream_t s, const PairGramItem* d_items, int nitems, int total_wgs);

}
```

### tensornetworkquantumsimulator.jl_amd/csrc/kernels_mfma.hip

```cpp
#include "kernels.hpp"
#include "mfma_common.hpp"
#include <stdexcept>
#include <type_traits>
#include "launch_util.hpp"

namespace tnqs {

template <int KB, int NB, int NU>
__global__ __launch_bounds__(256) void mfma_fiber_gemm_w_kernel(const FiberItem* __restrict__ items, int nitems,
                                                                double* __restrict__ norm_partials) {
    constexpr int KKP = 32 * KB, NNP = 32 * NB;
    constexpr int CP = (KKP > NNP ? KKP : NNP);
    constexpr int PT = CP + 1, PX = KKP + 1;
    extern __shared__ __attribute__((aligned(16))) char smem[];
    float* Xt_re = reinterpret_cast<float*>(smem);
    float* Xt_im = Xt_re + NNP * PX;
    const int tid = threadIdx.x, lane = tid & 63, w = tid >> 6, ln = lane & 31, h = lane >> 5;
    float* At_re = Xt_im + NNP * PX + w * (2 * 32 * PT);
    float* At_im = At_re + 32 * PT;
    __shared__ double sh_red[4];
    const int gw = blockIdx.x;
    const int lo = find_item(items, nitems, &FiberItem::tile_begin, gw);
    const FiberItem it = items[lo];
    const int D = it.D, K = it.K, TA = it.TA, TB = it.TB, KK = D * K;
// ... 238 lines not shown
            for (int e = tid; e < ntile_el; e += 256) {
                int s = e % D; int r1 = e / D; int al = r1 % TA; int r2 = r1 / TA; int k = r2 % K; int bl = r2 / K;
                cf vx, vy; vx.re = vx.im = vy.re = vy.im = 0.f;
                if (al < na && bl < nb) {
                    long long off = s + D * ((long long)(a0 + al) + PA * ((long long)k + (long long)K * (b0 + bl)));
                    vx = Xg[off]; vy = same ? vx : Yg[off];
                }
                int o = (s + D * k) * TRP + (al + TA * bl);
                Xr[o] = vx.re; Xi[o] = vx.im; Yr[o] = vy.re; Yi[o] = vy.im;
            }
        }
        lds_barrier();
        if (fast && t + 1 < t_end) issue_loads(t + 1);
        float xr[8], xi[8], yr[8], yi[8];
        const int ro = ln * TRP + 16 * w + 8 * h;
#pragma unroll
        for (int q = 0; q < 2; ++q) {
            v4f t0 = *reinterpret_cast<const v4f*>(Xr + ro + 4 * q), t1 = *reinterpret_cast<const v4f*>(Xi + ro + 4 * q);
            v4f t2 = *reinterpret_cast<const v4f*>(Yr + ro + 4 * q), t3 = *reinterpret_cast<const v4f*>(Yi + ro + 4 * q);
#pragma unroll
            for (int c = 0; c < 4; ++c) { xr[4 * q + c] = t0[c]; xi[4 * q + c] = t1[c]; yr[4 * q + c] = t2[c]; yi[4 * q + c] = t3[c]; }
        }
#pragma unroll
        for (int q = 0; q < 8; ++q) {
            Cr = __builtin_amdgcn_mfma_f32_32x32x2f32(xr[q], yr[q], Cr, 0, 0, 0);
            Cr = __builtin_amdgcn_mfma_f32_32x32x2f32(xi[q], yi[q], Cr, 0, 0, 0);
            Ci = __builtin_amdgcn_mfma_f32_32x32x2f32(xi[q], yr[q], Ci, 0, 0, 0);
            Ci = __builtin_amdgcn_mfma_f32_32x32x2f32(-xr[q], yi[q], Ci, 0, 0, 0);
        }
    }
    cf* __restrict__ part = reinterpret_cast<cf*>(it.partial) + (size_t)(4 * lc + w) * KK * KK;
#pragma unroll
    for (int r = 0; r < 16; ++r) {
        int i = (r & 3) + 8 * (r >> 2) + 4 * h, j = ln;
        if (i < KK && j < KK) { cf v; v.re = Cr[r]; v.im = Ci[r]; part[i + (size_t)KK * j] = v; }
    }
}
__global__ __launch_bounds__(256) void mfma_gram32_fused_kernel(const GramItem* __restrict__ items, int nitems) {
    constexpr int PITCH = 65, NU = 16;
    extern __shared__ __attribute__((aligned(16))) char smem[];
    const int tid = threadIdx.x, lane = tid & 63, w = tid >> 6, ln = lane & 31, h = lane >> 5;
    float* Lr = reinterpret_cast<float*>(smem) + w * (2 * 32 * PITCH);
    float* Li = Lr + 32 * PITCH;
    const int gc = blockIdx.x;
    const int lo = find_item(items, nitems, &GramItem::chunk_begin, gc);
    const GramItem it = items[lo];
    const int lc = gc - it.chunk_begin;
    const int K = it.K, TA = it.TA, TB = it.TB;
    const long long PA = it.PA;
    const cf* __restrict__ Xg = reinterpret_cast<const cf*>(it.X);
    const cf* __restrict__ Yg = reinterpret_cast<const cf*>(it.Y);
    const cf* __restrict__ Mg = reinterpret_cast<const cf*>(it.M);
    const int ntiles = it.nta * it.ntb;
    const int t_begin = lc * it.tiles_per_chunk;
    const int t_end = min(ntiles, t_begin + it.tiles_per_chunk);
    float mr[16], mi[16];
#pragma unroll
    for (int q = 0; q < 16; ++q) { cf v = Mg[(q + 16 * h) + 32 * ln]; mr[q] = v.re; mi[q] = v.im; }
    for (int e = lane; e < 32 * PITCH; e += 64) { Lr[e] = 0.f; Li[e] = 0.f; }
    v16f Or, Oi;
#pragma unroll
    for (int r = 0; r < 16; ++r) { Or[r] = 0.f; Oi[r] = 0.f; }
    const TileMap m = make_map(lane, 1, TA, TB, PA, K, 64);
    const long long kstride = PA;
    v4f pre[NU];
    auto issue = [&](const cf* __restrict__ G, int t) {
        int ta = t % it.nta, tb = t / it.nta;
        int a0 = ta * TA, b0 = tb * TB;
        const long long org = a0 + PA * (long long)K * b0;
#pragma unroll
        for (int j = 0; j < NU; ++j) {
            int k = m.kp + m.KP * j;
            v4f v; v[0] = v[1] = v[2] = v[3] = 0.f;
            if (k < K) v = ldg4(G + org + m.off + kstride * k);
            pre[j] = v;
        }
    };
    auto commit = [&]() {
#pragma unroll
        for (int j = 0; j < NU; ++j) {
            int k = m.kp + m.KP * j;
            if (k < K) { int o0 = k * PITCH + m.row0; Lr[o0] = pre[j][0]; Li[o0] = pre[j][1]; Lr[o0 + 1] = pre[j][2]; Li[o0 + 1] = pre[j][3]; }
        }
    };
    const int t_first = t_begin + w;
    if (t_first < t_end) issue(Xg, t_first);
    for (int t = t_first; t < t_end; t += 4) {
        commit();
        __builtin_amdgcn_wave_barrier();
        issue(Yg, t);
        v16f C1r[2], C1i[2];
#pragma unroll
        for (int s = 0; s < 2; ++s) {
            float xr[16], xi[16];
#pragma unroll
            for (int q = 0; q < 16; ++q) { int o = ln * PITCH + s + 2 * (q + 16 * h); xr[q] = Lr[o]; xi[q] = Li[o]; }
#pragma unroll
            for (int r = 0; r < 16; ++r) { C1r[s][r] = 0.f; C1i[s][r] = 0.f; }
#pragma unroll
            for (int q = 0; q < 16; ++q) {
                C1r[s] = __builtin_amdgcn_mfma_f32_32x32x2f32(mr[q], xr[q], C1r[s], 0, 0, 0);
                C1r[s] = __builtin_amdgcn_mfma_f32_32x32x2f32(-mi[q], xi[q], C1r[s], 0, 0, 0);
                C1i[s] = __builtin_amdgcn_mfma_f32_32x32x2f32(mr[q], xi[q], C1i[s], 0, 0, 0);
                C1i[s] = __builtin_amdgcn_mfma_f32_32x32x2f32(mi[q], xr[q], C1i[s], 0, 0, 0);
            }
        }
        __builtin_amdgcn_wave_barrier();
        commit();
        __builtin_amdgcn_wave_barrier();
        if (t + 4 < t_end) issue(Xg, t + 4);
#pragma unroll
        for (int s = 0; s < 2; ++s) {
            float yr[16], yi[16];
#pragma unroll
            for (int r = 0; r < 16; ++r) { int j = (r & 3) + 8 * (r >> 2) + 4 * h; int o = ln * PITCH + s + 2 * j; yr[r] = Lr[o]; yi[r] = Li[o]; }
#pragma unroll
            for (int r = 0; r < 16; ++r) {
                Or = __builtin_amdgcn_mfma_f32_32x32x2f32(C1r[s][r], yr[r], Or, 0, 0, 0);
                Or = __builtin_amdgcn_mfma_f32_32x32x2f32(C1i[s][r], yi[r], Or, 0, 0, 0);
                Oi = __builtin_amdgcn_mfma_f32_32x32x2f32(C1i[s][r], yr[r], Oi, 0, 0, 0);
                Oi = __builtin_amdgcn_mfma_f32_32x32x2f32(-C1r[s][r], yi[r], Oi, 0, 0, 0);
            }
        }
        __builtin_amdgcn_wave_barrier();
    }
    cf* __restrict__ part = reinterpret_cast<cf*>(it.partial) + (size_t)(4 * lc + w) * K * K;
#pragma unroll
    for (int r = 0; r < 16; ++r) {
        int i = (r & 3) + 8 * (r >> 2) + 4 * h, j = ln;
        if (i < K && j < K) { cf v; v.re = Or[r]; v.im = Oi[r]; part[i + (size_t)K * j] = v; }
    }
}
void launch_mfma_gram32_fused(hipStream_t s, const GramItem* d_items, int nitems, int total_chunks) {
    if (total_chunks <= 0) return;
    const size_t lds = (size_t)4 * 2 * 32 * 65 * sizeof(float);
    set_max_dynamic_lds((const void*)mfma_gram32_fused_kernel, lds);
    hipLaunchKernelGGL(mfma_gram32_fused_kernel, dim3(total_chunks), dim3(256), lds, s, d_items, nitems); TNQS_CHECK_LAUNCH();
}

__device__ __forceinline__ long long pair_slice_base(const PairGeom& g, int sl) {
    int a0 = sl % g.n0; int r1 = sl / g.n0; int a1 = r1 % g.n1; int a2 = r1 / g.n1;
    return (long long)a0 * g.t0 + (long long)a1 * g.t1 + (long long)a2 * g.t2;
}
__global__ __launch_bounds__(512) __attribute__((amdgpu_waves_per_eu(2, 2))) void mfma_pair_kernel(const PairItem* __restrict__ items, int nitems) {
    constexpr int PS = 32 * 33 + 4;
    constexpr int BUF = 8 * PS;
    #define TNQS_PIN() __builtin_amdgcn_sched_barrier(0x2 | 0x4)
    extern __shared__ __attribute__((aligned(16))) char smem[];
    v2f* L = reinterpret_cast<v2f*>(smem);
    const int tid = threadIdx.x, lane = tid & 63, w = tid >> 6, ln = lane & 31, h = lane >> 5;
    const int gw = blockIdx.x;
    const int lo = find_item(items, nitems, &PairItem::slice_begin, gw);
    const PairItem it = items[lo];
    const PairGeom g = it.g;
    const int nslices = g.n0 * g.n1 * g.n2;
    const int lw = gw - it.slice_begin;
    const int half = (lw >> 3) & 1, pw = ((lw >> 4) << 3) | (lw & 7);
    const int s_begin = pw * it.spw, s_end = min(nslices, s_begin + it.spw);
    const cf* __restrict__ in = reinterpret_cast<const cf*>(it.in);
    cf* __restrict__ out = reinterpret_cast<cf*>(it.out);
    float mxr[16], mxi[16], myr[16], myi[16];
    {
        const cf* __restrict__ Mx = reinterpret_cast<const cf*>(it.Mx) + 32 * ln; const cf* __restrict__ My = reinterpret_cast<const cf*>(it.My) + 32 * ln;
#pragma unroll
        for (int q = 0; q < 16; q += 2) { const v4f v = ldg4(Mx + q + 16 * h); mxr[q] = v[0]; mxi[q] = v[1]; mxr[q + 1] = v[2]; mxi[q + 1] = v[3]; }
#pragma unroll
        for (int q = 0; q < 16; q += 4) {
            const v4f u = ldg4(My + 2 * q + 4 * h), v = ldg4(My + 2 * q + 4 * h + 2);
            myr[q] = u[0]; myi[q] = u[1]; myr[q + 1] = u[2]; myi[q + 1] = u[3]; myr[q + 2] = v[0]; myi[q + 2] = v[1]; myr[q + 3] = v[2]; myi[q + 3] = v[3];
        }
    }
    const int f4 = tid & 3, sg0 = tid >> 2;
    const int ix0 = sg0 & 31, iy0 = sg0 >> 5;
    const long long toff = (long long)(4 * half + f4) * g.cstr + g.sx * ix0 + g.sy * iy0, tstr = 4 * g.sy;
    v2f* const lbase = L + (2 * f4) * PS + iy0 * 33 + ix0;
    v4f pre[8];
    auto commit = [&](int buf) {
#pragma unroll
        for (int j = 0; j < 8; ++j) {
            v2f* p0 = lbase + buf * BUF + 132 * j;
            v2f a; a[0] = pre[j][0]; a[1] = pre[j][1]; v2f b; b[0] = pre[j][2]; b[1] = pre[j][3];
            p0[0] = a; p0[PS] = b;
        }
    };
    auto store1 = [&](int buf, long long ob, int j) {
        const v2f* p0 = lbase + buf * BUF + 132 * j;
        const v2f a = p0[0], c = p0[PS];
        v4f v; v[0] = a[0]; v[1] = a[1]; v[2] = c[0]; v[3] = c[1];
        stg4(out + ob + tstr * j, v);
    };
    if (s_begin < s_end) {
        const long long b = pair_slice_base(g, s_begin) + toff;
#pragma unroll
        for (int j = 0; j < 8; ++j) pre[j] = ldg4(in + b + tstr * j);
        commit(0);
    }
    lds_barrier();
    for (int sl = s_begin; sl < s_end; ++sl) {
        const int buf = (sl - s_begin) & 1;
        const bool more = sl + 1 < s_end, prev = sl > s_begin;
        const long long nb = pair_slice_base(g, more ? sl + 1 : sl) + toff;
        const long long ob = pair_slice_base(g, prev ? sl - 1 : sl) + toff;
        v2f* P = L + buf * BUF + w * PS;
        v2f xc[4], xn[4];
#pragma unroll
        for (int i = 0; i < 4; ++i) xc[i] = P[ln * 33 + i + 16 * h];
        CAcc32<true> Y;
#pragma unroll
        for (int c4 = 0; c4 < 4; ++c4) {
            if (c4 < 3) {
#pragma unroll
                for (int i = 0; i < 4; ++i) xn[i] = P[ln * 33 + 4 * (c4 + 1) + i + 16 * h];
            }
            TNQS_PIN();
#pragma unroll
            for (int i = 0; i < 4; ++i) {
                const int q = 4 * c4 + i;
                const float br = mxr[q], bi = mxi[q];
                if (q == 0) Y.template mac_bpre<true>(xc[i][0], xc[i][1], br, bi - br, br + bi);
                else Y.template mac_bpre<false>(xc[i][0], xc[i][1], br, bi - br, br + bi);
                if ((q & 1) == 0) { pre[q >> 1] = ldg4(in + nb + tstr * (q >> 1)); TNQS_PIN(); }
            }
#pragma unroll
            for (int i = 0; i < 4; ++i) xc[i] = xn[i];
        }
        CAcc32<true> S;
#pragma unroll
        for (int r = 0; r < 16; ++r) {
            const float br = myr[r], bi = myi[r];
            if (r == 0) S.template mac_bpre<true>(Y.re(r), Y.im(r), br, bi - br, br + bi);
            else S.template mac_bpre<false>(Y.re(r), Y.im(r), br, bi - br, br + bi);
            if ((r & 1) == 0) { if (prev) store1(buf ^ 1, ob, r >> 1); TNQS_PIN(); }
        }
        S.finish();
#pragma unroll
        for (int r = 0; r < 16; ++r) { const int jx = (r & 3) + 8 * (r >> 2) + 4 * h; v2f v; v[0] = S.a[r]; v[1] = S.b[r]; P[ln * 33 + jx] = v; }
        if (more) commit(buf ^ 1);
        lds_barrier();
    }
    if (s_begin < s_end) {
        const int buf = (s_end - 1 - s_begin) & 1;
        const long long ob = pair_slice_base(g, s_end - 1) + toff;
#pragma unroll
        for (int j = 0; j < 8; ++j) store1(buf, ob, j);
    }
    #undef TNQS_PIN
}
static int pair_slices(const PairGeom& g) { return g.n0 * g.n1 * g.n2; }
int plan_pair(PairItem* it, int n, int spw) {
    if (spw <= 0) {
        double tot = 0; for (int i = 0; i < n; ++i) tot += pair_slices(it[i].g); spw = 16; while (spw > 1 && 2.0 * tot / spw < 1024.0) spw >>= 1;
    }
    return lay_out(it, n, &PairItem::slice_begin, nullptr, [&](PairItem& p) { p.spw = spw; const int np = (pair_slices(p.g) + spw - 1) / spw; return 16 * ((np + 7) / 8); });
}
void launch_mfma_pair(hipStream_t s, const PairItem* d_items, int nitems, int total_wgs) {
    if (total_wgs <= 0) return;
    if (mfma_use_x3()) { launch_x3_pair(s, d_items, nitems, total_wgs); return; }
    const size_t lds = (size_t)16 * (32 * 33 + 4) * 2 * sizeof(float);
    set_max_dynamic_lds((const void*)mfma_pair_kernel, lds); hipLaunchKernelGGL(mfma_pair_kernel, dim3(total_wgs), dim3(512), lds, s, d_items, nitems);
    TNQS_CHECK_LAUNCH();
}

__global__ __launch_bounds__(512) void mfma_pair_gram_kernel(const PairGramItem* __restrict__ items, int nitems) {
    constexpr int PS = 32 * 33 + 1;
    extern __shared__ __attribute__((aligned(16))) char smem[];
    v2f* L = reinterpret_cast<v2f*>(smem);
    const int tid = threadIdx.x, lane = tid & 63, w = tid >> 6, ln = lane & 31, h = lane >> 5;
    const int gw = blockIdx.x;
    const int lo = find_item(items, nitems, &PairGramItem::wg_begin, gw);
    const PairGramItem it = items[lo];
    const PairGeom g = it.g;
    const int nslices = g.n0 * g.n1 * g.n2;
    const int lw = gw - it.wg_begin;
    const int s_begin = lw * it.spw, s_end = min(nslices, s_begin + it.spw);
    const cf* __restrict__ Xg = reinterpret_cast<const cf*>(it.X);
    const cf* __restrict__ Yg = reinterpret_cast<const cf*>(it.Y);
    const cf* __restrict__ Mg = reinterpret_cast<const cf*>(it.M);
    float mr[16], mi[16];
#pragma unroll
    for (int q = 0; q < 16; ++q) { cf v = Mg[(q + 16 * h) + 32 * ln]; mr[q] = v.re; mi[q] = v.im; }
    v16f Or, Oi;
#pragma unroll
    for (int r = 0; r < 16; ++r) { Or[r] = 0.f; Oi[r] = 0.f; }
    const int f = tid & 7, sg0 = tid >> 3;
    const long long sx = g.sx, sy = g.sy, fo = (long long)f * g.cstr;
    v4f pre[16];
    const int ix0 = sg0 & 31, iy0 = sg0 >> 5;
    const long long toff = fo + sx * ix0 + sy * iy0, tstr = 2 * sy;
    v2f* const lbase = L + (2 * f) * PS + iy0 * 33 + ix0;
    auto issue = [&](const cf* __restrict__ G, int sl) {
        const cf* p = G + pair_slice_base(g, sl) + toff;
#pragma unroll
        for (int j = 0; j < 16; ++j) pre[j] = ldg4(p + tstr * j);
    };
    auto commit = [&]() {
#pragma unroll
        for (int j = 0; j < 16; ++j) {
            v2f* p0 = lbase + 66 * j;
            v2f a; a[0] = pre[j][0]; a[1] = pre[j][1]; v2f b; b[0] = pre[j][2]; b[1] = pre[j][3];
            p0[0] = a; p0[PS] = b;
        }
    };

    if (s_begin < s_end) issue(Xg, s_begin);
    for (int sl = s_begin; sl < s_end; ++sl) {
        lds_barrier();
        commit();
        lds_barrier();
        issue(Yg, sl);
        v16f C1r[2], C1i[2];
#pragma unroll
        for (int pp = 0; pp < 2; ++pp) {
            const v2f* P = L + (w + 8 * pp) * PS;
            float xr[16], xi[16];
#pragma unroll
            for (int q = 0; q < 16; ++q) { v2f v = P[ln * 33 + q + 16 * h]; xr[q] = v[0]; xi[q] = v[1]; }
#pragma unroll
            for (int r = 0; r < 16; ++r) { C1r[pp][r] = 0.f; C1i[pp][r] = 0.f; }
#pragma unroll
            for (int q = 0; q < 16; ++q) {
                C1r[pp] = __builtin_amdgcn_mfma_f32_32x32x2f32(mr[q], xr[q], C1r[pp], 0, 0, 0);
                C1r[pp] = __builtin_amdgcn_mfma_f32_32x32x2f32(-mi[q], xi[q], C1r[pp], 0, 0, 0);
                C1i[pp] = __builtin_amdgcn_mfma_f32_32x32x2f32(mr[q], xi[q], C1i[pp], 0, 0, 0);
                C1i[pp] = __builtin_amdgcn_mfma_f32_32x32x2f32(mi[q], xr[q], C1i[pp], 0, 0, 0);
            }
        }
        lds_barrier();
        commit();
        lds_barrier();
        if (sl + 1 < s_end) issue(Xg, sl + 1);
#pragma unroll
        for (int pp = 0; pp < 2; ++pp) {
            const v2f* P = L + (w + 8 * pp) * PS;
            float yr[16], yi[16];
#pragma unroll
            for (int r = 0; r < 16; ++r) { int jx = (r & 3) + 8 * (r >> 2) + 4 * h; v2f v = P[ln * 33 + jx]; yr[r] = v[0]; yi[r] = v[1]; }
#pragma unroll
            for (int r = 0; r < 16; ++r) {
                Or = __builtin_amdgcn_mfma_f32_32x32x2f32(C1r[pp][r], yr[r], Or, 0, 0, 0);
                Or = __builtin_amdgcn_mfma_f32_32x32x2f32(C1i[pp][r], yi[r], Or, 0, 0, 0);
                Oi = __builtin_amdgcn_mfma_f32_32x32x2f32(C1i[pp][r], yr[r], Oi, 0, 0, 0);
                Oi = __builtin_amdgcn_mfma_f32_32x32x2f32(-C1r[pp][r], yi[r], Oi, 0, 0, 0);
            }
        }
    }
    cf* __restrict__ part = reinterpret_cast<cf*>(it.partial) + (size_t)lw * 1024;
    v2f* const R = L;
    lds_barrier();
#pragma unroll
    for (int r = 0; r < 16; ++r) {
        const int i = (r & 3) + 8 * (r >> 2) + 4 * h;
        v2f v; v[0] = Or[r]; v[1] = Oi[r];
        R[w * (32 * 33) + ln * 33 + i] = v;
    }
    lds_barrier();
    for (int e = threadIdx.x; e < 1024; e += 512) {
        const int i = e & 31, j = e >> 5;
        float sr = 0.f, si = 0.f;
#pragma unroll
        for (int ww = 0; ww < 8; ++ww) { const v2f v = R[ww * (32 * 33) + j * 33 + i]; sr += v[0]; si += v[1]; }
        cf o; o.re = sr; o.im = si; part[e] = o;
    }
}
int plan_pair_gram(PairGramItem* it, int n, int* nwg, int spw) {
    if (spw <= 0) { double tot = 0; for (int i = 0; i < n; ++i) tot += pair_slices(it[i].g); spw = (int)std::max(4.0, std::min(16.0, tot / 2048.0)); }
    return lay_out(it, n, &PairGramItem::wg_begin, nwg, [&](PairGramItem& p) { p.spw = spw; return (pair_slices(p.g) + spw - 1) / spw; });
}
void launch_mfma_pair_gram(hipStream_t s, const PairGramItem* d_items, int nitems, int total_wgs) {
    if (total_wgs <= 0) return;
    const size_t lds = (size_t)16 * (32 * 33 + 1) * 2 * sizeof(float);
    set_max_dynamic_lds((const void*)mfma_pair_gram_kernel, lds);
    hipLaunchKernelGGL(mfma_pair_gram_kernel, dim3(total_wgs), dim3(512), lds, s, d_items, nitems); TNQS_CHECK_LAUNCH();
}

__global__ __launch_bounds__(512) __attribute__((amdgpu_waves_per_eu(2, 2))) void mfma_pair_gram2_kernel(const PairGram2Item* __restrict__ items, int nitems) {
    constexpr int PS = 32 * 33 + 8;
    constexpr int BUF = 8 * PS;
    #define TNQS_PIN() __builtin_amdgcn_sched_barrier(0x2 | 0x4)
    extern __shared__ __attribute__((aligned(16))) char smem[];
    v2f* L = reinterpret_cast<v2f*>(smem);
    const int tid = threadIdx.x, lane = tid & 63, w = tid >> 6, ln = lane & 31, h = lane >> 5;
    const int gw = blockIdx.x;
    const int lo = find_item(items, nitems, &PairGram2Item::wg_begin, gw);
    const PairGram2Item it = items[lo];
    const PairGeom g = it.g;
    const int nslices = g.n0 * g.n1 * g.n2;
    const int lw = gw - it.wg_begin;
    const int quarter = (lw >> 3) & 3, pw = ((lw >> 5) << 3) | (lw & 7);
    const int s_begin = pw * it.spw, s_end = min(nslices, s_begin + it.spw);
    const cf* __restrict__ Xg = reinterpret_cast<const cf*>(it.X);
    const cf* __restrict__ Yg = reinterpret_cast<const cf*>(it.Y);
    const int comp = w & 3, msg = w >> 2;
    float m0[16], mr[16], mi[16];
    {
        const cf* __restrict__ M = reinterpret_cast<const cf*>(msg ? it.My : it.Mx) + 16 * h + 32 * ln;
#pragma unroll
        for (int q = 0; q < 16; q += 2) { const v4f v = ldg4(M + q); mr[q] = v[0]; mi[q] = v[1]; mr[q + 1] = v[2]; mi[q + 1] = v[3]; }
#pragma unroll
        for (int q = 0; q < 16; ++q) m0[q] = mr[q] + mi[q];
    }
    const int f2 = tid & 1, sg0 = tid >> 1;
    const int ix0 = sg0 & 31, iy0 = sg0 >> 5;
    const long long toff = (long long)(2 * quarter + f2) * g.cstr + g.sx * ix0 + g.sy * iy0, tstr = 8 * g.sy;
    v2f* const lbase = L + (2 * f2) * PS + iy0 * 33 + ix0;
    v4f px[4], py[4];
    auto commit = [&](int buf) {
#pragma unroll
        for (int j = 0; j < 4; ++j) {
            v2f* p0 = lbase + buf * BUF + 264 * j;
            v2f a; a[0] = px[j][0]; a[1] = px[j][1]; v2f b; b[0] = px[j][2]; b[1] = px[j][3];
            p0[0] = a; p0[PS] = b;
            v2f c; c[0] = py[j][0]; c[1] = py[j][1]; v2f d; d[0] = py[j][2]; d[1] = py[j][3];
            p0[4 * PS] = c; p0[5 * PS] = d;
        }
    };
    CAcc32<true> O; O.zero();
    if (s_begin < s_end) {
        const long long b = pair_slice_base(g, s_begin) + toff;
#pragma unroll
        for (int j = 0; j < 4; ++j) { px[j] = ldg4(Xg + b + tstr * j); py[j] = ldg4(Yg + b + tstr * j); }
        commit(0);
    }
    lds_barrier();
    auto run = [&](auto msg_c) {
    constexpr int MSG = decltype(msg_c)::value;
    for (int sl = s_begin; sl < s_end; ++sl) {
        const int buf = (sl - s_begin) & 1;
        const bool more = sl + 1 < s_end;
        const v2f* PX = L + buf * BUF + comp * PS; const v2f* PY = PX + 4 * PS;
        const long long nb = pair_slice_base(g, more ? sl + 1 : sl) + toff;
        auto xat = [&](int k) { return MSG ? PX[k * 33 + ln] : PX[ln * 33 + k]; };
        auto yat = [&](int k) { return MSG ? PY[k * 33 + ln] : PY[ln * 33 + k]; };
        v2f xc[4], xn[4];
#pragma unroll
        for (int i = 0; i < 4; ++i) xc[i] = xat(i + 16 * h);
        CAcc32<true> C;
#pragma unroll
        for (int c4 = 0; c4 < 4; ++c4) {
#pragma unroll
            for (int i = 0; i < 4; ++i) {
                if (c4 < 3) xn[i] = xat(4 * (c4 + 1) + i + 16 * h);
                else { const int r = i, k = (r & 3) + 8 * (r >> 2) + 4 * h; xn[i] = yat(k); }
            }
            TNQS_PIN();
#pragma unroll
            for (int i = 0; i < 4; ++i) {
                const int q = 4 * c4 + i;
                if (q == 0) C.template mac_pre<true>(m0[q], mr[q], mi[q], xc[i][0], xc[i][1]);
                else C.template mac_pre<false>(m0[q], mr[q], mi[q], xc[i][0], xc[i][1]);
                if ((q & 1) == 0) {
                    const int j = q >> 2;
                    if ((q & 2) == 0) px[j] = ldg4(Xg + nb + tstr * j); else py[j] = ldg4(Yg + nb + tstr * j);
                    TNQS_PIN();
                }
            }
#pragma unroll
            for (int i = 0; i < 4; ++i) xc[i] = xn[i];
        }
#pragma unroll
        for (int c4 = 0; c4 < 4; ++c4) {
            if (c4 < 3) {
#pragma unroll
                for (int i = 0; i < 4; ++i) { const int r = 4 * (c4 + 1) + i, k = (r & 3) + 8 * (r >> 2) + 4 * h; xn[i] = yat(k); }
            }
            TNQS_PIN();
#pragma unroll
            for (int i = 0; i < 4; ++i) {
                const int r = 4 * c4 + i;
                O.mac_conj(C.re(r), C.im(r), xc[i][0], xc[i][1]);
            }
#pragma unroll
            for (int i = 0; i < 4; ++i) xc[i] = xn[i];
        }
        if (more) commit(buf ^ 1);
        lds_barrier();
    }
    };
    if (msg == 0) run(std::integral_constant<int, 0>{}); else run(std::integral_constant<int, 1>{});
    O.finish_conj();
    cf* __restrict__ p1 = reinterpret_cast<cf*>(it.partial_y) + (size_t)lw * 1024;
    cf* __restrict__ p2 = reinterpret_cast<cf*>(it.partial_x) + (size_t)lw * 1024;
    v2f* const R = L;
#pragma unroll
    for (int r = 0; r < 16; ++r) {
        const int i = (r & 3) + 8 * (r >> 2) + 4 * h;
        v2f v; v[0] = O.a[r]; v[1] = O.b[r];
        R[w * (32 * 33) + ln * 33 + i] = v;
    }
    lds_barrier();
    for (int e = tid; e < 2048; e += 512) {
        const int mm = e >> 10, ee = e & 1023, i = ee & 31, j = ee >> 5;
        float sr = 0.f, si = 0.f;
#pragma unroll
        for (int ww = 0; ww < 4; ++ww) { const v2f v = R[(4 * mm + ww) * (32 * 33) + j * 33 + i]; sr += v[0]; si += v[1]; }
        cf o; o.re = sr; o.im = si; stgc((mm ? p2 : p1) + ee, o);
    }
    #undef TNQS_PIN
}
int x3_pair_gram2_group();
int plan_pair_gram2(PairGram2Item* it, int n, int* nwg, int spw) {
    auto groups = [](const PairGram2Item& p, int w) { const int np = (pair_slices(p.g) + w - 1) / w; return (np + 7) / 8; };
    if (spw <= 0)
        for (spw = 16; spw > 1; spw >>= 1) { long tot = 0; for (int i = 0; i < n; ++i) tot += 16 * groups(it[i], spw); if (tot >= 1024) break; }
    const int per_group = mfma_use_x3() ? x3_pair_gram2_group() : 32;
    return lay_out(it, n, &PairGram2Item::wg_begin, nwg, [&](PairGram2Item& p) { p.spw = spw; return per_group * groups(p, spw); });
}
void launch_mfma_pair_gram2(hipStream_t s, const PairGram2Item* d_items, int nitems, int total_wgs) {
    if (total_wgs <= 0) return;
    if (mfma_use_x3()) { launch_x3_pair_gram2(s, d_items, nitems, total_wgs); return; }
    const size_t lds = (size_t)16 * (32 * 33 + 8) * 2 * sizeof(float);
    set_max_dynamic_lds((const void*)mfma_pair_gram2_kernel, lds);
    hipLaunchKernelGGL(mfma_pair_gram2_kernel, dim3(total_wgs), dim3(512), lds, s, d_items, nitems);
    TNQS_CHECK_LAUNCH();
}

__global__ __launch_bounds__(256) void recover_v_mfma_kernel(const RecoverItem* __restrict__ items) {
    const RecoverItem it = items[blockIdx.x];
    if (it.pre && theta_pre_takes(it.dyn, it.dm, it.dn, it.pre == 2)) return;
    const cf* __restrict__ A0 = reinterpret_cast<const cf*>(it.A0);
    const cf* __restrict__ A = reinterpret_cast<const cf*>(it.A);
    cf* __restrict__ V = reinterpret_cast<cf*>(it.V);
    int m_ = it.m, n_ = it.n, nu_ = it.nu;
    if (it.dyn) theta_dims(it.dyn, it.dm, it.dn, m_, n_, nu_);
    const int m = m_, n = n_, nu = nu_;
    const int lane = threadIdx.x & 63, w = threadIdx.x >> 6, ln = lane & 31, h = lane >> 5;
    const int nt = (n + 31) >> 5;
    const int tile = blockIdx.y * 4 + w;
    if (tile >= nt * nt || n < 1 || nu < 1) return;
    const int c0 = 32 * (tile % nt), u0 = 32 * (tile / nt);
    const int col = c0 + ln, u = u0 + ln;
    const cf* pa = A0 + (size_t)m * min(col, n - 1);
    const cf* pb = A + (size_t)m * min(u, nu - 1);
    if (u0 >= nu) return;
    const bool okc = col < n, oku = u < nu;
    v16f Cr, Ci;
#pragma unroll
    for (int r = 0; r < 16; ++r) { Cr[r] = 0.f; Ci[r] = 0.f; }
    double s2 = 0.0;
    for (int k0 = 0; k0 < m; k0 += 2) {
        const int row = k0 + h;
        cf a = {0.f, 0.f}, b = {0.f, 0.f};
        if (row < m) { if (okc) a = pa[row]; if (oku) b = pb[row]; }
        s2 += (double)b.re * b.re + (double)b.im * b.im;
        Cr = __builtin_amdgcn_mfma_f32_32x32x2f32(a.re, b.re, Cr, 0, 0, 0);
        Cr = __builtin_amdgcn_mfma_f32_32x32x2f32(a.im, b.im, Cr, 0, 0, 0);
        Ci = __builtin_amdgcn_mfma_f32_32x32x2f32(a.re, b.im, Ci, 0, 0, 0);
        Ci = __builtin_amdgcn_mfma_f32_32x32x2f32(-a.im, b.re, Ci, 0, 0, 0);
    }
    s2 += __shfl_xor(s2, 32, 64);
    const double inv = s2 > 0.0 ? 1.0 / s2 : 0.0;
    if (oku) {
#pragma unroll
        for (int r = 0; r < 16; ++r) {
            int c = c0 + (r & 3) + 8 * (r >> 2) + 4 * h;
            if (c < n) { cf v; v.re = (float)(Cr[r] * inv); v.im = (float)(Ci[r] * inv); V[c + (size_t)n * u] = v; }
        }
    }
}
void launch_recover_v_mfma(hipStream_t s, const RecoverItem* d_items, int nitems, int nmax) {
    if (nitems <= 0) return;
    const int nt = (nmax + 31) / 32;
    hipLaunchKernelGGL(recover_v_mfma_kernel, dim3(nitems, (nt * nt + 3) / 4), dim3(256), 0, s, d_items); TNQS_CHECK_LAUNCH();
}

template <bool SHARED>
__global__ __launch_bounds__(256, 2) void mfma_gram64_f64_kernel(const GramItem* __restrict__ items, int nitems) {
    constexpr int TR = 64, TRP = TR + 4, NU = 8;
    extern __shared__ __attribute__((aligned(16))) char smem[];
    float* const Xbuf = reinterpret_cast<float*>(smem);
    const int tid = threadIdx.x;
    const int gc = blockIdx.x;
    const int lo = find_item(items, nitems, &GramItem::chunk_begin, gc);
    const GramItem it = items[lo];
    const int lc = gc - it.chunk_begin;
    const int D = it.D, K = it.K, TA = it.TA, TB = it.TB, KK = D * K;
    const long long PA = it.PA;
    const cf* __restrict__ Xg = reinterpret_cast<const cf*>(it.X);
    const int ntiles = it.nta * it.ntb;
    const int t_begin = lc * it.tiles_per_chunk;
    const int t_end = min(ntiles, t_begin + it.tiles_per_chunk);
    const int lane = tid & 63, w = tid >> 6, l15 = lane & 15, kq = lane >> 4;
    const int nb = (KK + 15) >> 4, nblk = nb * (nb + 1) / 2;
    const int parA = (w < 2) ? 0 : 1;
    int aI[3], aJ[3], bI[2], bJ[2]; bool aOn[3], bOn[2];
    auto block_of = [&](int idx, int& I, int& J) { I = 0; int rem = idx; while (rem >= nb - I) { rem -= nb - I; ++I; } J = I + rem; };
#pragma unroll
    for (int q = 0; q < 3; ++q) { const int wv = parA ? 3 - w : w; int idx = wv + 4 * q; aOn[q] = idx < nblk; block_of(aOn[q] ? idx : 0, aI[q], aJ[q]); }
#pragma unroll
    for (int q = 0; q < 2; ++q) { const int wv = parA ? w : 3 - w; int idx = wv + 4 * q; bOn[q] = idx < nblk; block_of(bOn[q] ? idx : 0, bI[q], bJ[q]); }
    constexpr bool shared_sets = SHARED;
    if (shared_sets) {
#pragma unroll
        for (int q = 0; q < 3; ++q) { aOn[q] = true; aI[q] = (w & 1) ? q : 0; aJ[q] = (w & 1) ? 3 : q; }
        bOn[0] = bOn[1] = true;
        bI[0] = (w & 1) ? 2 : 1; bJ[0] = (w & 1) ? 2 : 1; bI[1] = (w & 1) ? 3 : 1; bJ[1] = (w & 1) ? 3 : 2;
    }
    v4d CAr[3], CAi[3], CBr[2], CBi[2], CAc[3], CBc[2];
#pragma unroll
    for (int j = 0; j < 3; ++j)
#pragma unroll
        for (int r = 0; r < 4; ++r) { CAr[j][r] = 0.0; CAi[j][r] = 0.0; CAc[j][r] = 0.0; }
#pragma unroll
    for (int j = 0; j < 2; ++j)
#pragma unroll
        for (int r = 0; r < 4; ++r) { CBr[j][r] = 0.0; CBi[j][r] = 0.0; CBc[j][r] = 0.0; }
    for (int e = tid; e < 4 * 64 * TRP; e += 256) Xbuf[e] = 0.f;
    const TileMap m = make_map(tid, D, TA, TB, PA, K);
    const long long kstride = (long long)D * PA;
    const bool fast = m.U <= 256 && (K + m.KP - 1) / m.KP <= NU;
    v4f px[NU];
    auto tile_origin = [&](int t, int& a0, int& b0, int& na, int& nb) {
        int ta = t % it.nta, tb = t / it.nta;
        a0 = ta * TA; b0 = tb * TB; na = min(TA, it.PA - a0); nb = min(TB, it.PB - b0);
    };
    const bool straight = fast && m.active && m.vec == 2 && K == m.KP * NU;
    auto issue_loads = [&](int t) {
        int a0, b0, na, nb; tile_origin(t, a0, b0, na, nb);
        const long long org = (long long)D * (a0 + PA * (long long)K * b0);
        if (straight && na == TA && nb == TB) {
            const cf* p0 = Xg + org + m.off + kstride * m.kp; const long long st = kstride * m.KP;
#pragma unroll
            for (int j = 0; j < NU; ++j) px[j] = ldg4(p0 + st * j);
            return;
        }
        const bool v0 = m.active && m.al < na && m.bl < nb, v1 = v0 && m.al1 < na;
#pragma unroll
        for (int j = 0; j < NU; ++j) {
            int k = m.kp + m.KP * j;
            v4f vx; vx[0] = vx[1] = vx[2] = vx[3] = 0.f;
            if (k < K && v0) {
                const long long o = org + m.off + kstride * k;
                if (m.vec == 2 && v1) vx = ldg4(Xg + o);
                else { cf x = ldgc(Xg + o); vx[0] = x.re; vx[1] = x.im; }
            }
            px[j] = vx;
        }
    };
    auto commit_loads = [&](int buf) {
        if (!m.active) return;
        float* Xr = Xbuf + buf * (2 * 64 * TRP); float* Xi = Xr + 64 * TRP;
#pragma unroll
        for (int j = 0; j < NU; ++j) {
            int k = m.kp + m.KP * j;
            if (k < K) {
                int o0 = (m.c0 + D * k) * TRP + m.row0;
                Xr[o0] = px[j][0]; Xi[o0] = px[j][1];
                if (m.vec == 2) { int o1 = (m.c1 + D * k) * TRP + m.row1; Xr[o1] = px[j][2]; Xi[o1] = px[j][3]; }
            }
        }
    };
    auto fill_slow = [&](int t, int buf) {
        float* Xr = Xbuf + buf * (2 * 64 * TRP); float* Xi = Xr + 64 * TRP;
        int a0, b0, na, nb; tile_origin(t, a0, b0, na, nb);
// ... 103 lines not shown
```

### tensornetworkquantumsimulator.jl_amd/csrc/kernels_x3.hip

```cpp
#include <type_traits>
#include "kernels.hpp"
#include "mfma_common.hpp"
#include "launch_util.hpp"
#include "x3_common.hpp"

namespace tnqs {

__device__ __forceinline__ long long x3_slice_base(const PairGeom& g, int sl) {
    int a0 = sl % g.n0; int r1 = sl / g.n0; int a1 = r1 % g.n1; int a2 = r1 / g.n1;
    return (long long)a0 * g.t0 + (long long)a1 * g.t1 + (long long)a2 * g.t2;
}

template <bool SINGLE>
__global__ __launch_bounds__(512) __attribute__((amdgpu_waves_per_eu(2, 2))) void x3_pair_gram2_kernel(const PairGram2Item* __restrict__ items, int nitems) {
    constexpr int P = 34;
    constexpr int PS = 32 * P + 2;
    #define TNQS_PIN() __builtin_amdgcn_sched_barrier(0x2 | 0x4)
    extern __shared__ __attribute__((aligned(16))) char smem[];
    v2f* L = reinterpret_cast<v2f*>(smem);
    const int tid = threadIdx.x, lane = tid & 63, w = tid >> 6, ln = lane & 31, h = lane >> 5;
    const int gw = blockIdx.x;
    const int lo = find_item(items, nitems, &PairGram2Item::wg_begin, gw);
    const PairGram2Item it = items[lo];
    const PairGeom g = it.g;
    const int nslices = g.n0 * g.n1 * g.n2;
    const int lw = gw - it.wg_begin;
    const int half = (lw >> 3) & 1, pw = ((lw >> 4) << 3) | (lw & 7);
    const int s_begin = pw * it.spw, s_end = min(nslices, s_begin + it.spw);
    const cf* __restrict__ Xg = reinterpret_cast<const cf*>(it.X);
    const cf* __restrict__ Yg = reinterpret_cast<const cf*>(it.Y);
    const int comp = SINGLE ? w : (w & 3), msg = SINGLE ? 0 : (w >> 2);
    P3 Mr[2], Mi[2];
    {
        const cf* __restrict__ M = reinterpret_cast<const cf*>(msg ? it.My : it.Mx) + 32 * ln + 8 * h;
#pragma unroll
        for (int n = 0; n < 2; ++n) {
            float xr[8], xi[8];
#pragma unroll
            for (int e = 0; e < 8; e += 2) { const v4f v = ldg4(M + 16 * n + e); xr[e] = v[0]; xi[e] = v[1]; xr[e + 1] = v[2]; xi[e + 1] = v[3]; }
            Mr[n] = split8(xr); Mi[n] = split8(xi);
        }
    }
    const int f4 = tid & 3, sg0 = tid >> 2;
    const int ix0 = sg0 & 31, iy0 = sg0 >> 5;
    const long long toff = (long long)(4 * half + f4) * g.cstr + g.sx * ix0 + g.sy * iy0, tstr = 4 * g.sy;
    v2f* const lbase = L + (2 * f4) * PS + iy0 * P + ix0;
    v4f px[8], py[8];
    auto commit = [&]() {
#pragma unroll
        for (int j = 0; j < 8; ++j) {
            v2f* p0 = lbase + 4 * P * j;
            v2f a; a[0] = px[j][0]; a[1] = px[j][1]; v2f b; b[0] = px[j][2]; b[1] = px[j][3];
            p0[0] = a; p0[PS] = b;
            v2f c; c[0] = py[j][0]; c[1] = py[j][1]; v2f d; d[0] = py[j][2]; d[1] = py[j][3];
            p0[8 * PS] = c; p0[9 * PS] = d;
        }
    };
    v16f Or, Oi;
#pragma unroll
    for (int r = 0; r < 16; ++r) { Or[r] = 0.f; Oi[r] = 0.f; }
    if (s_begin < s_end) {
        const long long b = x3_slice_base(g, s_begin) + toff;
#pragma unroll
        for (int j = 0; j < 8; ++j) { px[j] = ldg4(Xg + b + tstr * j); py[j] = ldg4(Yg + b + tstr * j); }
        commit();
    }
    lds_barrier();
    auto run = [&](auto msg_c) {
    constexpr int MSG = decltype(msg_c)::value;
    auto read8 = [&](const v2f* PL, int i0, int i1, float (&re)[8], float (&im)[8]) {
        if (MSG == 0) {
            const v4f* a = reinterpret_cast<const v4f*>(PL + ln * P + i0); const v4f* b = reinterpret_cast<const v4f*>(PL + ln * P + i1);
            const v4f a0 = a[0], a1 = a[1], b0 = b[0], b1 = b[1];
            re[0] = a0[0]; im[0] = a0[1]; re[1] = a0[2]; im[1] = a0[3]; re[2] = a1[0]; im[2] = a1[1]; re[3] = a1[2]; im[3] = a1[3];
            re[4] = b0[0]; im[4] = b0[1]; re[5] = b0[2]; im[5] = b0[3]; re[6] = b1[0]; im[6] = b1[1]; re[7] = b1[2]; im[7] = b1[3];
        } else {
#pragma unroll
            for (int e = 0; e < 4; ++e) { const v2f u = PL[(i0 + e) * P + ln], v = PL[(i1 + e) * P + ln]; re[e] = u[0]; im[e] = u[1]; re[4 + e] = v[0]; im[4 + e] = v[1]; }
        }
    };
    for (int sl = s_begin; sl < s_end; ++sl) {
        const bool more = sl + 1 < s_end;
        const long long nb = x3_slice_base(g, more ? sl + 1 : sl) + toff;
        float ar[8], ai[8], br[8], bi[8];
        read8(L + comp * PS, 8 * h, 8 * h + 4, ar, ai);
#pragma unroll
        for (int t = 0; t < (SINGLE ? 1 : 2); ++t) {
            const v2f* PX = L + (comp + 4 * t) * PS; const v2f* PY = PX + 8 * PS;
            v16f Cr, Ci;
            read8(PX, 16 + 8 * h, 16 + 8 * h + 4, br, bi);
            if (t == 0) {
#pragma unroll
                for (int j = 0; j < 2; ++j) { px[j] = ldg4(Xg + nb + tstr * j); py[j] = ldg4(Yg + nb + tstr * j); }
            }
            TNQS_PIN();
            {
                const P3 xr = split8(ar), xi = split8(ai);
                mac6x2<true>(Cr, Mr[0], xr, Ci, Mr[0], xi);
                mac6x2<false>(Cr, Mi[0], neg(xi), Ci, Mi[0], xr);
            }
            read8(PY, 4 * h, 4 * h + 8, ar, ai);
            if (t == 0) {
#pragma unroll
                for (int j = 2; j < 4; ++j) { px[j] = ldg4(Xg + nb + tstr * j); py[j] = ldg4(Yg + nb + tstr * j); }
            }
            TNQS_PIN();
            {
                const P3 xr = split8(br), xi = split8(bi);
                mac6x2<false>(Cr, Mr[1], xr, Ci, Mr[1], xi);
                mac6x2<false>(Cr, Mi[1], neg(xi), Ci, Mi[1], xr);
            }
            read8(PY, 16 + 4 * h, 16 + 4 * h + 8, br, bi);
            if (t == 0) {
#pragma unroll
                for (int j = 4; j < 6; ++j) { px[j] = ldg4(Xg + nb + tstr * j); py[j] = ldg4(Yg + nb + tstr * j); }
            }
            TNQS_PIN();
            {
                float cr[8], ci[8];
#pragma unroll
                for (int e = 0; e < 8; ++e) { cr[e] = Cr[e]; ci[e] = Ci[e]; }
                const P3 pcr = split8(cr), pci = split8(ci), yr = split8(ar), yi = split8(ai);
                mac6x2<false>(Or, pcr, yr, Oi, pci, yr);
                mac6x2<false>(Or, pci, yi, Oi, neg(pcr), yi);
            }
            if (t == 0) {
#pragma unroll
                for (int j = 6; j < 8; ++j) { px[j] = ldg4(Xg + nb + tstr * j); py[j] = ldg4(Yg + nb + tstr * j); }
            }
            if (t == 0 && !SINGLE) read8(L + (comp + 4) * PS, 8 * h, 8 * h + 4, ar, ai);
            TNQS_PIN();
            {
                float cr[8], ci[8];
#pragma unroll
                for (int e = 0; e < 8; ++e) { cr[e] = Cr[8 + e]; ci[e] = Ci[8 + e]; }
                const P3 pcr = split8(cr), pci = split8(ci), yr = split8(br), yi = split8(bi);
                mac6x2<false>(Or, pcr, yr, Oi, pci, yr);
                mac6x2<false>(Or, pci, yi, Oi, neg(pcr), yi);
            }
        }
        TNQS_PIN();
        lds_barrier();
        if (more) commit();
        lds_barrier();
    }
    };
    if (SINGLE || msg == 0) run(std::integral_constant<int, 0>{}); else run(std::integral_constant<int, 1>{});
    cf* __restrict__ p1 = reinterpret_cast<cf*>(it.partial_y) + (size_t)lw * 1024;
    cf* __restrict__ p2 = reinterpret_cast<cf*>(it.partial_x) + (size_t)lw * 1024;
    v2f* const R = L;
#pragma unroll
    for (int r = 0; r < 16; ++r) {
        const int i = (r & 3) + 8 * (r >> 2) + 4 * h;
        v2f v; v[0] = Or[r]; v[1] = Oi[r];
        R[w * (32 * 33) + ln * 33 + i] = v;
    }
    lds_barrier();
    if (SINGLE) {
        for (int e = tid; e < 1024; e += 512) {
            const int i = e & 31, j = e >> 5;
            float sr = 0.f, si = 0.f;
#pragma unroll
            for (int ww = 0; ww < 8; ++ww) { const v2f v = R[ww * (32 * 33) + j * 33 + i]; sr += v[0]; si += v[1]; }
            cf o; o.re = sr; o.im = si; stgc(p1 + e, o);
        }
        return;
    }
    for (int e = tid; e < 2048; e += 512) {
        const int mm = e >> 10, ee = e & 1023, i = ee & 31, j = ee >> 5;
        float sr = 0.f, si = 0.f;
#pragma unroll
        for (int ww = 0; ww < 4; ++ww) { const v2f v = R[(4 * mm + ww) * (32 * 33) + j * 33 + i]; sr += v[0]; si += v[1]; }
        cf o; o.re = sr; o.im = si; stgc((mm ? p2 : p1) + ee, o);
    }
}
#undef TNQS_PIN
int x3_pair_gram2_group() { return 16; }
int plan_x3_pair_gram1(PairGram2Item* it, int n, int* nwg, int spw) {
    auto slices = [](const PairGram2Item& p) { return p.g.n0 * p.g.n1 * p.g.n2; };
    if (spw <= 0) { double tot = 0; for (int i = 0; i < n; ++i) tot += (double)slices(it[i]); spw = 16; while (spw > 1 && 2.0 * tot / spw < 1024.0) spw >>= 1; }
    return lay_out(it, n, &PairGram2Item::wg_begin, nwg, [&](PairGram2Item& p) { p.spw = spw; const int np = (slices(p) + spw - 1) / spw; return 16 * ((np + 7) / 8); });
}
void launch_x3_pair_gram1(hipStream_t s, const PairGram2Item* d_items, int nitems, int total_wgs) {
    if (total_wgs <= 0) return;
    const size_t lds = (size_t)16 * (32 * 34 + 2) * 2 * sizeof(float);
    set_max_dynamic_lds((const void*)x3_pair_gram2_kernel<true>, lds);
    hipLaunchKernelGGL((x3_pair_gram2_kernel<true>), dim3(total_wgs), dim3(512), lds, s, d_items, nitems);
    TNQS_CHECK_LAUNCH();
}
void launch_x3_pair_gram2(hipStream_t s, const PairGram2Item* d_items, int nitems, int total_wgs) {
    if (total_wgs <= 0) return;
    const size_t lds = (size_t)16 * (32 * 34 + 2) * 2 * sizeof(float);
    set_max_dynamic_lds((const void*)x3_pair_gram2_kernel<false>, lds);
    hipLaunchKernelGGL(x3_pair_gram2_kernel<false>, dim3(total_wgs), dim3(512), lds, s, d_items, nitems);
    TNQS_CHECK_LAUNCH();
}

__global__ __launch_bounds__(512) __attribute__((amdgpu_waves_per_eu(2, 2))) void x3_pair_kernel(const PairItem* __restrict__ items, int nitems) {
    constexpr int P = 34;
    constexpr int PS = 32 * P + 2;
    constexpr int BUF = 8 * PS;
    extern __shared__ __attribute__((aligned(16))) char smem[];
    v2f* L = reinterpret_cast<v2f*>(smem);
    const int tid = threadIdx.x, lane = tid & 63, w = tid >> 6, ln = lane & 31, h = lane >> 5;
    const int gw = blockIdx.x;
    const int lo = find_item(items, nitems, &PairItem::slice_begin, gw);
    const PairItem it = items[lo];
    const PairGeom g = it.g;
    const int nslices = g.n0 * g.n1 * g.n2;
    const int lw = gw - it.slice_begin;
    const int half = (lw >> 3) & 1, pw = ((lw >> 4) << 3) | (lw & 7);
    const int s_begin = pw * it.spw, s_end = min(nslices, s_begin + it.spw);
    const cf* __restrict__ in = reinterpret_cast<const cf*>(it.in);
    cf* __restrict__ out = reinterpret_cast<cf*>(it.out);
    P3 Mxr[2], Mxi[2];
    u4* const MyL = reinterpret_cast<u4*>(L + 16 * PS) + lane;
    {
        const cf* __restrict__ Mx = reinterpret_cast<const cf*>(it.Mx) + 32 * ln; const cf* __restrict__ My = reinterpret_cast<const cf*>(it.My) + 32 * ln;
#pragma unroll
        for (int n = 0; n < 2; ++n) {
            float xr[8], xi[8];
#pragma unroll
            for (int e = 0; e < 8; e += 2) { const v4f v = ldg4(Mx + 16 * n + 8 * h + e); xr[e] = v[0]; xi[e] = v[1]; xr[e + 1] = v[2]; xi[e + 1] = v[3]; }
            Mxr[n] = split8(xr); Mxi[n] = split8(xi);
#pragma unroll
            for (int e = 0; e < 8; e += 2) { const v4f v = ldg4(My + 4 * h + 16 * n + 8 * (e >> 2) + (e & 3)); xr[e] = v[0]; xi[e] = v[1]; xr[e + 1] = v[2]; xi[e + 1] = v[3]; }
            const P3 yr_ = split8(xr), yi_ = split8(xi);
            if (w == 0) { MyL[(6 * n + 0) * 64] = yr_.h; MyL[(6 * n + 1) * 64] = yr_.m; MyL[(6 * n + 2) * 64] = yr_.l; MyL[(6 * n + 3) * 64] = yi_.h; MyL[(6 * n + 4) * 64] = yi_.m; MyL[(6 * n + 5) * 64] = yi_.l; }
        }
    }
    const int f4 = tid & 3, sg0 = tid >> 2;
    const int ix0 = sg0 & 31, iy0 = sg0 >> 5;
    const long long toff = (long long)(4 * half + f4) * g.cstr + g.sx * ix0 + g.sy * iy0, tstr = 4 * g.sy;
    v2f* const lbase = L + (2 * f4) * PS + iy0 * P + ix0;
    v4f preA[8], preB[8];
    #define TNQS_PIN() __builtin_amdgcn_sched_barrier(0x2 | 0x4)
    auto commit = [&](int buf, const v4f (&pre)[8]) {
#pragma unroll
        for (int j = 0; j < 8; ++j) {
            v2f* p0 = lbase + buf * BUF + 4 * P * j;
            v2f a; a[0] = pre[j][0]; a[1] = pre[j][1]; v2f b; b[0] = pre[j][2]; b[1] = pre[j][3];
            p0[0] = a; p0[PS] = b;
        }
    };
    auto store1 = [&](int buf, long long ob, int j) {
        const v2f* p0 = lbase + buf * BUF + 4 * P * j;
        const v2f a = p0[0], c = p0[PS];
        v4f v; v[0] = a[0]; v[1] = a[1]; v[2] = c[0]; v[3] = c[1];
        stg4(out + ob + tstr * j, v);
    };
    if (s_begin < s_end) {
        const long long b = x3_slice_base(g, s_begin) + toff;
#pragma unroll
        for (int j = 0; j < 8; ++j) preB[j] = ldg4(in + b + tstr * j);
        const long long b1 = x3_slice_base(g, s_begin + 1 < s_end ? s_begin + 1 : s_begin) + toff;
#pragma unroll
        for (int j = 0; j < 8; ++j) preA[j] = ldg4(in + b1 + tstr * j);
        commit(0, preB);
    }
    lds_barrier();
    auto phase = [&](int sl, int buf, const v4f (&cur)[8], v4f (&nxt)[8]) {
        const bool more = sl + 1 < s_end, prev = sl > s_begin;
        const long long nb = x3_slice_base(g, sl + 2 < s_end ? sl + 2 : sl) + toff;
        const long long ob = x3_slice_base(g, prev ? sl - 1 : sl) + toff;
        v2f* Pw = L + buf * BUF + w * PS;
        v16f Yr, Yi;
#pragma unroll
        for (int n = 0; n < 2; ++n) {
            float ar[8], ai[8];
            const v4f* a = reinterpret_cast<const v4f*>(Pw + ln * P + 16 * n + 8 * h);
#pragma unroll
            for (int q = 0; q < 4; ++q) { const v4f v = a[q]; ar[2 * q] = v[0]; ai[2 * q] = v[1]; ar[2 * q + 1] = v[2]; ai[2 * q + 1] = v[3]; }
#pragma unroll
            for (int j = 0; j < 4; ++j) nxt[4 * n + j] = ldg4(in + nb + tstr * (4 * n + j));
            TNQS_PIN();
            const P3 sr = split8(ar), si = split8(ai), nsi = neg(si);
            if (n == 0) mac6x2<true>(Yr, sr, Mxr[n], Yi, sr, Mxi[n]); else mac6x2<false>(Yr, sr, Mxr[n], Yi, sr, Mxi[n]);
            mac6x2<false>(Yr, nsi, Mxi[n], Yi, si, Mxr[n]);
        }
        v16f Sr, Si;
#pragma unroll
        for (int n = 0; n < 2; ++n) {
            float yr[8], yi[8];
#pragma unroll
            for (int e = 0; e < 8; ++e) { yr[e] = Yr[8 * n + e]; yi[e] = Yi[8 * n + e]; }
            const P3 pr = split8(yr), pi = split8(yi), npi = neg(pi);
            if (prev) {
#pragma unroll
                for (int j = 0; j < 4; ++j) store1(buf ^ 1, ob, 4 * n + j);
            }
            P3 myr, myi;
            myr.h = MyL[(6 * n + 0) * 64]; myr.m = MyL[(6 * n + 1) * 64]; myr.l = MyL[(6 * n + 2) * 64]; myi.h = MyL[(6 * n + 3) * 64]; myi.m = MyL[(6 * n + 4) * 64]; myi.l = MyL[(6 * n + 5) * 64];
            TNQS_PIN();
            if (n == 0) mac6x2<true>(Sr, pr, myr, Si, pr, myi); else mac6x2<false>(Sr, pr, myr, Si, pr, myi);
            mac6x2<false>(Sr, npi, myi, Si, pi, myr);
        }
        TNQS_PIN();
#pragma unroll
        for (int r = 0; r < 16; r += 2) { const int jx = (r & 3) + 8 * (r >> 2) + 4 * h; v4f v; v[0] = Sr[r]; v[1] = Si[r]; v[2] = Sr[r + 1]; v[3] = Si[r + 1]; *reinterpret_cast<v4f*>(Pw + ln * P + jx) = v; }
        if (more) commit(buf ^ 1, cur);
        lds_barrier();
    };
    for (int sl = s_begin; sl < s_end; sl += 2) {
        phase(sl, 0, preA, preB);
        if (sl + 1 < s_end) phase(sl + 1, 1, preB, preA);
    }
    if (s_begin < s_end) {
        const int buf = (s_end - 1 - s_begin) & 1;
        const long long ob = x3_slice_base(g, s_end - 1) + toff;
#pragma unroll
        for (int j = 0; j < 8; ++j) store1(buf, ob, j);
    }
    #undef TNQS_PIN
}
void launch_x3_pair(hipStream_t s, const PairItem* d_items, int nitems, int total_wgs) {
    if (total_wgs <= 0) return;
    const size_t lds = (size_t)16 * (32 * 34 + 2) * 2 * sizeof(float) + 12 * 64 * 16;
    set_max_dynamic_lds((const void*)x3_pair_kernel, lds);
    hipLaunchKernelGGL(x3_pair_kernel, dim3(total_wgs), dim3(512), lds, s, d_items, nitems);
    TNQS_CHECK_LAUNCH();
}

template <int D>
__global__ __launch_bounds__(256, 2) void x3_rowgemm64_kernel(const FiberItem* __restrict__ items, int nitems, double* __restrict__ norm_partials) {
    constexpr int KK = 64;
    extern __shared__ __attribute__((aligned(16))) char smem[];
    u4* const Xl = reinterpret_cast<u4*>(smem);
    __shared__ double sh_red[4];
    const int tid = threadIdx.x, lane = tid & 63, w = tid >> 6, ln = lane & 31, h = lane >> 5;
    const int gw = blockIdx.x;
    const int lo = find_item(items, nitems, &FiberItem::tile_begin, gw);
    const FiberItem it = items[lo];
    const int K = it.K, No = it.No, NN = it.Do * No;
    const long long PA = it.PA;
    const int ntiles = it.nta * it.ntb;
    const int t_begin = (gw - it.tile_begin) * it.tpw, t_end = min(ntiles, t_begin + it.tpw);
    const cf* __restrict__ in = reinterpret_cast<const cf*>(it.in);
    const cf* __restrict__ X = reinterpret_cast<const cf*>(it.X);
    cf* __restrict__ out = reinterpret_cast<cf*>(it.out);
    for (int e = tid; e < 4 * 2 * 64; e += 256) {
        const int l = e & 63, nb = (e >> 6) & 1, n = e >> 7;
        const int nn = 32 * nb + (l & 31), kk0 = 16 * n + 8 * (l >> 5);
        float xr[8], xi[8];
#pragma unroll
        for (int q = 0; q < 8; q += 2) {
            v4f v = {0.f, 0.f, 0.f, 0.f};
            if (nn < NN) v = ldg4(X + kk0 + q + (size_t)KK * nn);
            xr[q] = v[0]; xi[q] = v[1]; xr[q + 1] = v[2]; xi[q + 1] = v[3];
        }
        const P3 pr = split8(xr), pi = split8(xi);
        u4* d = Xl + (size_t)((2 * n + nb) * 6) * 64 + l;
        d[0] = pr.h; d[64] = pr.m; d[128] = pr.l; d[192] = pi.h; d[256] = pi.m; d[320] = pi.l;
    }
    __syncthreads();
    float hb[2][32];
    const bool rows_b = PA < 32;
    const int RB = rows_b ? 32 / (int)PA : 1;
    const long long kst = (long long)D * PA;
    const long long lane_in = rows_b ? (long long)D * (ln % (int)PA) + kst * K * (ln / (int)PA) : (long long)D * ln;
    const long long lane_out = rows_b ? (long long)D * (ln % (int)PA) + kst * No * (ln / (int)PA) : (long long)D * ln;
    auto base_in = [&](int t) { return rows_b ? kst * K * RB * t : (long long)D * 32 * (t % it.nta) + kst * K * (t / it.nta); };
    auto base_out = [&](int t) { return rows_b ? kst * No * RB * t : (long long)D * 32 * (t % it.nta) + kst * No * (t / it.nta); };
    const unsigned voff = (unsigned)((lane_in + kst * (D == 1 ? 8 : 4) * h) * (long long)sizeof(cf));
    auto issue_half = [&](int t, int hf) {
        const cf* pu = in + base_in(t);
#pragma unroll
        for (int nn2 = 0; nn2 < 2; ++nn2) {
            const int n = 2 * hf + nn2;
            if (D == 1) {
#pragma unroll
                for (int e = 0; e < 8; ++e) { const v2f v = ldg2(reinterpret_cast<const char*>(pu + kst * (16 * n + e)) + voff); hb[hf][16 * nn2 + e] = v[0]; hb[hf][16 * nn2 + 8 + e] = v[1]; }
            } else {
#pragma unroll
                for (int j = 0; j < 4; ++j) { const v4f v = ldg4(reinterpret_cast<const char*>(pu + kst * (8 * n + j)) + voff);
                                              hb[hf][16 * nn2 + 2 * j] = v[0]; hb[hf][16 * nn2 + 8 + 2 * j] = v[1]; hb[hf][16 * nn2 + 2 * j + 1] = v[2]; hb[hf][16 * nn2 + 8 + 2 * j + 1] = v[3]; }
            }
        }
    };
    double nrm = 0;
    int t = t_begin + w;
    if (t < t_end) { issue_half(t, 0); issue_half(t, 1); }
    for (; t < t_end; t += 4) {
        v16f Cr[2], Ci[2];
#pragma unroll
        for (int hf = 0; hf < 2; ++hf) {
#pragma unroll
            for (int nn2 = 0; nn2 < 2; ++nn2) {
                const int n = 2 * hf + nn2;
                float br[8], bi[8];
#pragma unroll
                for (int e = 0; e < 8; ++e) { br[e] = hb[hf][16 * nn2 + e]; bi[e] = hb[hf][16 * nn2 + 8 + e]; }
                const P3 pbr = split8(br), pbi = split8(bi), nbi = neg(pbi);
#pragma unroll
                for (int nb = 0; nb < 2; ++nb) {
                    const u4* a = Xl + (size_t)((2 * n + nb) * 6) * 64 + lane;
                    P3 xr, xi; xr.h = a[0]; xr.m = a[64]; xr.l = a[128]; xi.h = a[192]; xi.m = a[256]; xi.l = a[320];
                    if (n == 0) mac6x2<true>(Cr[nb], xr, pbr, Ci[nb], xr, pbi); else mac6x2<false>(Cr[nb], xr, pbr, Ci[nb], xr, pbi);
                    mac6x2<false>(Cr[nb], xi, nbi, Ci[nb], xi, pbr);
                }
            }
            __builtin_amdgcn_sched_barrier(0);
            if (t + 4 < t_end) issue_half(t + 4, hf);
        }
        float nf = 0.f;
        cf* p = out + base_out(t) + lane_out;
        if (D == 1) {
#pragma unroll
            for (int nb = 0; nb < 2; ++nb)
#pragma unroll
                for (int r = 0; r < 16; ++r) {
                    const int n = 32 * nb + (r & 3) + 8 * (r >> 2) + 4 * h;
                    if (n < No) { cf v; v.re = Cr[nb][r]; v.im = Ci[nb][r]; stgc(p + PA * n, v); nf += v.re * v.re + v.im * v.im; }
                }
        } else {
#pragma unroll
            for (int nb = 0; nb < 2; ++nb)
#pragma unroll
                for (int r = 0; r < 16; r += 2) {
                    const int nn = 32 * nb + (r & 3) + 8 * (r >> 2) + 4 * h;
                    const int n = nn >> 1;
                    if (n < No) {
                        v4f v = {Cr[nb][r], Ci[nb][r], Cr[nb][r + 1], Ci[nb][r + 1]};
                        stg4(p + 2 * PA * n, v);
                        nf += v[0] * v[0] + v[1] * v[1] + v[2] * v[2] + v[3] * v[3];
                    }
                }
        }
        nrm += (double)nf;
    }
    if (it.want_norm) {
        nrm = wave_sum(nrm);
        if (lane == 0) sh_red[w] = nrm;
        __syncthreads();
        if (tid == 0) norm_partials[gw] = sh_red[0] + sh_red[1] + sh_red[2] + sh_red[3];
    }
}
void launch_x3_rowgemm64(hipStream_t s, const FiberItem* d_items, int nitems, int total_wgs, int D, double* d_norm_partials) {
    if (total_wgs <= 0) return;
    const size_t lds = (size_t)4 * 2 * 6 * 64 * 16;
    if (D == 1) { set_max_dynamic_lds((const void*)x3_rowgemm64_kernel<1>, lds); hipLaunchKernelGGL(x3_rowgemm64_kernel<1>, dim3(total_wgs), dim3(256), lds, s, d_items, nitems, d_norm_partials); }
    else { set_max_dynamic_lds((const void*)x3_rowgemm64_kernel<2>, lds); hipLaunchKernelGGL(x3_rowgemm64_kernel<2>, dim3(total_wgs), dim3(256), lds, s, d_items, nitems, d_norm_partials); }
    TNQS_CHECK_LAUNCH();
}

__global__ __launch_bounds__(256, 2) void x3_gram64_kernel(const GramItem* __restrict__ items, int nitems) {
    constexpr int TR = 64, TRP = TR + 4, NU = 8;
    extern __shared__ __attribute__((aligned(16))) char smem[];
    float* const Xr = reinterpret_cast<float*>(smem);
    float* const Xi = Xr + 64 * TRP;
    float* const Yr = Xi + 64 * TRP;
    float* const Yi = Yr + 64 * TRP;
    const int tid = threadIdx.x;
    const int gc = blockIdx.x;
    const int lo = find_item(items, nitems, &GramItem::chunk_begin, gc);
    const GramItem it = items[lo];
    const int lc = gc - it.chunk_begin;
    const int D = it.D, K = it.K, TA = it.TA, TB = it.TB, KK = D * K;
    const long long PA = it.PA;
    const bool same = (it.X == it.Y);
    const cf* __restrict__ Xg = reinterpret_cast<const cf*>(it.X);
    const cf* __restrict__ Yg = reinterpret_cast<const cf*>(it.Y);
    const int ntiles = it.nta * it.ntb;
// ... 139 lines not shown
```

Baseline: 6780.

## Write pair-kernel output in plane-major layout and read it via strided Gram geometry

Adds a separate output geometry to the chi = 32 pair kernels and a matching X-operand geometry to the pair-Gram kernels. When the shape qualifies, the pair product writes its intermediate tensor in a permuted, plane-major order chosen so the following Gram kernel reads it with friendlier strides. The goal is to cut strided or uncoalesced global traffic between the pair and Gram stages. It adds address arithmetic, an env switch to disable it, and debug entry points that check the permuted strides cover each element once.

```diff
diff --git a/include/tnqs_debug.h b/include/tnqs_debug.h
--- a/include/tnqs_debug.h
+++ b/include/tnqs_debug.h
@@ -38,6 +38,12 @@
                     int* route_out, int* spw_out, int* wg_begin_out, int* nwg_out, int* total_wgs_out);
 int tnqs_dbg_pair_gram32(int d, int nitems, const int* z, const int* chi, const int* lx, const int* ly, int form, const void* X, const void* Y, const void* M,
                          void* out_y, void* out_x, int spw, int guard, int* route_out, int* spw_out, int* wg_begin_out, int* nwg_out, int* total_wgs_out);
+int tnqs_dbg_pair_layout_plan(int d, const int* chi, int lx, int ly, int gx, int gy, int* covered, long long* out_strides, long long* x_strides,
+                              long long* pair_strides, int* pair_counts, long long* gram_strides, int* gram_counts);
+int tnqs_dbg_pair32_out(int d, int z, const int* chi, int lx, int ly, const long long* out_strides, const void* in, const void* M, void* out, int spw, int guard,
+                        int* route_out);
+int tnqs_dbg_pair_gram32_x(int d, int z, const int* chi, int lx, int ly, int form, const long long* x_strides, const void* X, const void* Y, const void* M,
+                           void* partials_y, void* partials_x, int spw, int* route_out, int* nwg_out);
 int tnqs_dbg_svd_tall(int nitems, const int* m, const int* n, void* A, int* chol_fail, int* polished, int* sweeps);
 int tnqs_dbg_small_site(int nitems, const int* d, const int* z, const int* chi, const int* jo, const void* psi, const void* M, const int* present, int form,
                         const void* old_msg, const int* has_old, int normalize, void* out, void* new_msg, double* diff_out, int* route_out);
diff --git a/tensornetworkquantumsimulator.jl_amd/csrc/debug_plane.cpp b/tensornetworkquantumsimulator.jl_amd/csrc/debug_plane.cpp
--- a/tensornetworkquantumsimulator.jl_amd/csrc/debug_plane.cpp
+++ b/tensornetworkquantumsimulator.jl_amd/csrc/debug_plane.cpp
@@ -385,3 +385,87 @@
         gOy.down(out_y, "out_y"); if (form == 0) gOx.down(out_x, "out_x");
     });
 }
+
+namespace {
+void geom_out(const PairGeom& g, long long* strides, int* counts) {
+    if (strides) { strides[0] = g.cstr; strides[1] = g.sx; strides[2] = g.sy; strides[3] = g.t0; strides[4] = g.t1; strides[5] = g.t2; }
+    if (counts) { counts[0] = g.n0; counts[1] = g.n1; counts[2] = g.n2; }
+}
+PairGeom strided(const char* who, const PairGeom& g, const long long* st, size_t n) {
+    if (!st) return g;
+    PairGeom q = g; q.cstr = st[0]; q.sx = st[1]; q.sy = st[2]; q.t0 = st[3]; q.t1 = st[4]; q.t2 = st[5];
+    std::vector<char> seen(n, 0);
+    for (int a2 = 0; a2 < q.n2; ++a2) for (int a1 = 0; a1 < q.n1; ++a1) for (int a0 = 0; a0 < q.n0; ++a0) for (int f = 0; f < 8; ++f) for (int iy = 0; iy < 32; ++iy) for (int ix = 0; ix < 32; ++ix) {
+        const long long o = a0 * q.t0 + a1 * q.t1 + a2 * q.t2 + f * q.cstr + ix * q.sx + iy * q.sy;
+        if (o < 0 || (o & 1) || (size_t)o + 1 >= n || seen[(size_t)o] || seen[(size_t)o + 1]) throw Err(TNQS_ERR_INVALID, std::string(who) + ": the strides do not enumerate the tensor once");
+        seen[(size_t)o] = seen[(size_t)o + 1] = 1;
+    }
+    return q;
+}
+}
+extern "C" int tnqs_dbg_pair_layout_plan(int d, const int* chi, int lx, int ly, int gx, int gy, int* covered, long long* out_strides, long long* x_strides,
+                                         long long* pair_strides, int* pair_counts, long long* gram_strides, int* gram_counts) {
+    return guard([&] {
+        if (!chi || !covered) throw Err(TNQS_ERR_INVALID, "dbg_pair_layout_plan: bad arguments");
+        PairGeom gp{}, gg{}, go{}, xg{};
+        if (!pair_geometry(d, 4, chi, lx, ly, gp) || !pair_geometry(d, 4, chi, gx, gy, gg)) throw Err(TNQS_ERR_UNSUPPORTED, "dbg_pair_layout_plan: shape not covered by the chi = 32 plane kernels");
+        *covered = use_plane_major_t() && plane_major_layout(d, chi, lx, ly, gx, gy, go, xg) ? 1 : 0;
+        if (!*covered) { go = gp; xg = gg; }
+        geom_out(go, out_strides, nullptr); geom_out(xg, x_strides, nullptr); geom_out(gp, pair_strides, pair_counts); geom_out(gg, gram_strides, gram_counts);
+    });
+}
+extern "C" int tnqs_dbg_pair32_out(int d, int z, const int* chi, int lx, int ly, const long long* out_strides, const void* in, const void* M, void* out, int spw, int guard_elems,
+                                   int* route) {
+    return guard([&] {
+        std::vector<PairGeom> g; std::vector<size_t> n;
+        pair32_geoms("dbg_pair32_out", d, 1, &z, chi, &lx, &ly, spw, guard_elems, g, n);
+        if (!in || !M || !out) throw Err(TNQS_ERR_INVALID, "dbg_pair32_out: bad arguments");
+        PairItem it{}; it.g = g[0]; it.go = strided("dbg_pair32_out", g[0], out_strides, n[0]);
+        const int wgs = plan_pair(&it, 1, spw);
+        if (route) *route = mfma_use_x3() ? TNQS_DBG_ROUTE_X3 : TNQS_DBG_ROUTE_F32;
+        need_gpu();
+        Slots sIn, sM; Guarded gO((size_t)guard_elems * 8);
+        sIn.add(n[0] * 8); sM.add(2 * 1024 * 8); gO.add(n[0] * 8);
+        alloc_all(sIn, sM, gO); put_all(sIn, in); put_all(sM, M);
+        it.in = sIn.at(0); it.out = gO.at(0); it.Mx = sM.at(0); it.My = sM.at(0) + 1024 * 8;
+        DevItems<PairItem> dI(1); dI.up(it);
+        up_all(sIn, sM); gO.up(out);
+        launch_mfma_pair(nullptr, dI.get(), 1, wgs);
+        HIPCHK(hipDeviceSynchronize());
+        gO.down(out, "out");
+    });
+}
+extern "C" int tnqs_dbg_pair_gram32_x(int d, int z, const int* chi, int lx, int ly, int form, const long long* x_strides, const void* X, const void* Y, const void* M,
+                                      void* partials_y, void* partials_x, int spw, int* route, int* nwg_out) {
+    return guard([&] {
+        std::vector<PairGeom> g; std::vector<size_t> n;
+        pair32_geoms("dbg_pair_gram32_x", d, 1, &z, chi, &lx, &ly, spw, 0, g, n);
+        if ((form != 0 && form != 1) || !nwg_out || (X && (!Y || !M || !partials_y || (form == 0 && !partials_x)))) throw Err(TNQS_ERR_INVALID, "dbg_pair_gram32_x: bad arguments");
+        const bool x3 = mfma_use_x3();
+        PairGram2Item two{}; PairGramItem one{};
+        two.g = one.g = g[0]; two.gx = one.gx = strided("dbg_pair_gram32_x", g[0], x_strides, n[0]);
+        int nwg = 0;
+        const int wgs = form == 0 ? plan_pair_gram2(&two, 1, &nwg, spw) : x3 ? plan_x3_pair_gram1(&two, 1, &nwg, spw) : plan_pair_gram(&one, 1, &nwg, spw);
+        *nwg_out = nwg;
+        if (route) *route = x3 ? TNQS_DBG_ROUTE_X3 : TNQS_DBG_ROUTE_F32;
+        if (!X) return;
+        need_gpu();
+        const size_t pb = (size_t)nwg * 1024 * 8;
+        Slots sX, sY, sM, sP(256);
+        sX.add(n[0] * 8); sY.add(n[0] * 8); sM.add(2 * 1024 * 8); sP.add(pb); if (form == 0) sP.add(pb);
+        alloc_all(sX, sY, sM, sP); put_all(sX, X); put_all(sY, Y); put_all(sM, M);
+        two.X = one.X = sX.at(0); two.Y = one.Y = sY.at(0); two.Mx = one.M = sM.at(0); two.My = form == 0 ? sM.at(0) + 1024 * 8 : nullptr;
+        two.partial_y = one.partial = sP.at(0); two.partial_x = form == 0 ? sP.at(1) : nullptr;
+        DevItems<PairGram2Item> dTwo(1); DevItems<PairGramItem> dOne(1); dTwo.up(two); dOne.up(one);
+        up_all(sX, sY, sM, sP);
+        if (form == 0) launch_mfma_pair_gram2(nullptr, dTwo.get(), 1, wgs);
+        else if (x3) launch_x3_pair_gram1(nullptr, dTwo.get(), 1, wgs);
+        else launch_mfma_pair_gram(nullptr, dOne.get(), 1, wgs);
+        HIPCHK(hipDeviceSynchronize());
+        sP.down("the pair-Gram partials");
+        auto untouched = [&](size_t b0, size_t b1) { for (size_t b = b0; b < b1; ++b) if (sP.host[b] != (char)0xff) throw Err(TNQS_ERR_INVALID, "dbg: a kernel wrote outside an item of the pair-Gram partials"); };
+        untouched(0, 256);
+        for (size_t k = 0; k < sP.off.size(); ++k) untouched(sP.off[k] + sP.len[k], sP.off[k] + sP.len[k] + 256);
+        sP.get(0, partials_y); if (form == 0) sP.get(1, partials_x);
+    });
+}
diff --git a/tensornetworkquantumsimulator.jl_amd/csrc/engine_bp.cpp b/tensornetworkquantumsimulator.jl_amd/csrc/engine_bp.cpp
--- a/tensornetworkquantumsimulator.jl_amd/csrc/engine_bp.cpp
+++ b/tensornetworkquantumsimulator.jl_amd/csrc/engine_bp.cpp
@@ -329,6 +329,7 @@
         const Buf& ma = u.incoming(src, pa, m.t); const Buf& mb = u.incoming(src, pb, m.t); const Buf& mr = u.incoming(src, r, m.t);
         PairGramItem gi{}; PairItem pi{};
         if (!(ma && mb && mr && pair_geometry(c.sd.d, c.sd.z, c.sd.chi.data(), pa, pb, pi.g) && pair_geometry(c.sd.d, c.sd.z, c.sd.chi.data(), r, jo, gi.g))) return false;
+        if (!(use_plane_major_t() && plane_major_layout(c.sd.d, c.sd.chi.data(), pa, pb, r, jo, pi.go, gi.gx))) { pi.go = pi.g; gi.gx = gi.g; }
         const int slot = std::min(pa, pb) < std::min(r, jo) ? 0 : 1;
         SharedT& sh = u.tshare[src][slot];
         if (!(sh.T && sh.site == s->site[src] && sh.ma == ma && sh.mb == mb && sh.la == pa && sh.lb == pb)) {
@@ -343,7 +344,7 @@
         auto pit = pend.find(key);
         if (pit != pend.end() && pit->second.jo == r && pit->second.r == jo && pair32_items[msgs[pit->second.msg].item].X == gi.X) {
             Msg& mf = msgs[pit->second.msg]; const PairGramItem& first = pair32_items[mf.item];
-            PairGram2Item d2{}; d2.X = first.X; d2.Y = first.Y; d2.Mx = first.M; d2.My = gi.M; d2.g = first.g;
+            PairGram2Item d2{}; d2.X = first.X; d2.Y = first.Y; d2.Mx = first.M; d2.My = gi.M; d2.g = first.g; d2.gx = first.gx;
             sh_dbl.push_back(d2); sh_dbl_msg.push_back({pit->second.msg, (int)msgs.size()});
             sh_dbl_slices += (double)c.sd.n / 8192.0;
             mf.route = m.route = Route::Pair32Double;
@@ -533,7 +534,7 @@
         if (singles.empty()) return;
         if (mfma_use_x3()) {
             std::vector<PairGram2Item> one(singles.size());
-            for (size_t q = 0; q < singles.size(); ++q) { const PairGramItem& a = singles[q]; one[q].X = a.X; one[q].Y = a.Y; one[q].Mx = a.M; one[q].g = a.g; }
+            for (size_t q = 0; q < singles.size(); ++q) { const PairGramItem& a = singles[q]; one[q].X = a.X; one[q].Y = a.Y; one[q].Mx = a.M; one[q].g = a.g; one[q].gx = a.gx; }
             launch_pair32_singles(one, &PairGram2Item::partial_y, single_msg, slices, plan_x3_pair_gram1, launch_x3_pair_gram1);
         } else launch_pair32_singles(singles, &PairGramItem::partial, single_msg, slices, plan_pair_gram, launch_mfma_pair_gram);
     }
diff --git a/tensornetworkquantumsimulator.jl_amd/csrc/engine_internal.hpp b/tensornetworkquantumsimulator.jl_amd/csrc/engine_internal.hpp
--- a/tensornetworkquantumsimulator.jl_amd/csrc/engine_internal.hpp
+++ b/tensornetworkquantumsimulator.jl_amd/csrc/engine_internal.hpp
@@ -29,6 +29,7 @@
 TNQS_SWITCH(use_pair, !envflag("TNQS_NO_PAIR"))
 TNQS_SWITCH(use_bra_products, !envflag("TNQS_NO_BRA_PRODUCTS"))
 TNQS_SWITCH(use_prodcache, !envflag("TNQS_NO_PRODCACHE"))
+TNQS_SWITCH(use_plane_major_t, !envflag("TNQS_NO_PLANE_MAJOR_T"))
 TNQS_SWITCH(use_chol, !envflag("TNQS_NO_CHOL"))
 TNQS_SWITCH(use_qr2, !envflag("TNQS_NO_QR2"))
 TNQS_SWITCH(use_lowrank, !envflag("TNQS_NO_LOWRANK"))
diff --git a/tensornetworkquantumsimulator.jl_amd/csrc/kernels.hpp b/tensornetworkquantumsimulator.jl_amd/csrc/kernels.hpp
--- a/tensornetworkquantumsimulator.jl_amd/csrc/kernels.hpp
+++ b/tensornetworkquantumsimulator.jl_amd/csrc/kernels.hpp
@@ -298,12 +298,14 @@
     PairGeom g;
     int slice_begin;
     int spw;
+    PairGeom go;
 };
 struct PairGramItem {
     const void* X; const void* Y; const void* M; void* partial;
     PairGeom g;
     int wg_begin;
     int spw;
+    PairGeom gx;
 };
 
 struct PlaneGeom { long long cstr, sx, sy, t0, t1, t2, t3; int n0, n1, n2, n3; int nslices() const { return n0 * n1 * n2 * n3; } };
@@ -339,6 +341,27 @@
     g = PairGeom{p.cstr, p.sx, p.sy, p.t0, p.t1, p.t2, p.n0, p.n1, p.n2};
     return true;
 }
+inline bool plane_major_layout(int d, const int* chi, int lx, int ly, int gx, int gy, PairGeom& out, PairGeom& xg) {
+    if (d != 2 || lx < 0 || ly > 3 || lx >= ly || gx < 0 || gy < 0 || gx > 3 || gy > 3 || gx == gy || gx == lx || gx == ly || gy == lx || gy == ly) return false;
+    for (int j = 0; j < 4; ++j) if (chi[j] != 32) return false;
+    PairGeom gp, gg;
+    if (!pair_geometry(d, 4, chi, lx, ly, gp) || !pair_geometry(d, 4, chi, gx, gy, gg)) return false;
+    long long ostr[4];
+    { long long st = 64; ostr[lx] = 2; for (int j = 0; j < 4; ++j) if (j != lx) { ostr[j] = st; st *= 32; } }
+    auto image = [&](long long off) { long long o = off % 2; off /= 2; for (int j = 0; j < 4; ++j) { o += (off % 32) * ostr[j]; off /= 32; } return o; };
+    auto permute = [&](const PairGeom& g, PairGeom& r) {
+        r = g;
+        r.cstr = image(g.cstr); r.sx = image(g.sx); r.sy = image(g.sy); r.t0 = image(g.t0); r.t1 = g.n1 > 1 ? image(g.t1) : 0; r.t2 = g.n2 > 1 ? image(g.t2) : 0;
+        bool ok = true;
+        for (int f = 0; f < 8; ++f) ok = ok && image(f * g.cstr) == f * r.cstr;
+        for (int i = 0; i < 32; ++i) ok = ok && image(i * g.sx) == i * r.sx && image(i * g.sy) == i * r.sy;
+        for (int a = 0; a < g.n0; ++a) ok = ok && image(a * g.t0) == a * r.t0;
+        for (int a = 0; a < g.n1; ++a) ok = ok && image(a * g.t1) == a * r.t1;
+        for (int a = 0; a < g.n2; ++a) ok = ok && image(a * g.t2) == a * r.t2;
+        return ok;
+    };
+    return permute(gp, out) && permute(gg, xg);
+}
 struct Pair16Item {
     const void* in; void* out; const void* Mx; const void* My;
     PlaneGeom g;
@@ -375,7 +398,7 @@
 int plan_pair(PairItem* it, int n, int spw = 0);
 void launch_mfma_pair(hipStream_t s, const PairItem* d_items, int nitems, int total_wgs);
 void launch_x3_pair(hipStream_t s, const PairItem* d_items, int nitems, int total_wgs);
-struct PairGram2Item { const void* X; const void* Y; const void* Mx; const void* My; void* partial_y; void* partial_x; PairGeom g; int wg_begin; int spw; };
+struct PairGram2Item { const void* X; const void* Y; const void* Mx; const void* My; void* partial_y; void* partial_x; PairGeom g; int wg_begin; int spw; PairGeom gx; };
 int plan_pair_gram2(PairGram2Item* it, int n, int* nwg = nullptr, int spw = 0);
 void launch_mfma_pair_gram2(hipStream_t s, const PairGram2Item* d_items, int nitems, int total_wgs);
 void launch_x3_pair_gram2(hipStream_t s, const PairGram2Item* d_items, int nitems, int total_wgs);
diff --git a/tensornetworkquantumsimulator.jl_amd/csrc/kernels_mfma.hip b/tensornetworkquantumsimulator.jl_amd/csrc/kernels_mfma.hip
--- a/tensornetworkquantumsimulator.jl_amd/csrc/kernels_mfma.hip
+++ b/tensornetworkquantumsimulator.jl_amd/csrc/kernels_mfma.hip
@@ -414,7 +414,7 @@
     const int gw = blockIdx.x;
     const int lo = find_item(items, nitems, &PairItem::slice_begin, gw);
     const PairItem it = items[lo];
-    const PairGeom g = it.g;
+    const PairGeom g = it.g, go = it.go;
     const int nslices = g.n0 * g.n1 * g.n2;
     const int lw = gw - it.slice_begin;
     const int half = (lw >> 3) & 1, pw = ((lw >> 4) << 3) | (lw & 7);
@@ -435,6 +435,7 @@
     const int f4 = tid & 3, sg0 = tid >> 2;
     const int ix0 = sg0 & 31, iy0 = sg0 >> 5;
     const long long toff = (long long)(4 * half + f4) * g.cstr + g.sx * ix0 + g.sy * iy0, tstr = 4 * g.sy;
+    const long long toffo = (long long)(4 * half + f4) * go.cstr + go.sx * ix0 + go.sy * iy0, tstro = 4 * go.sy;
     v2f* const lbase = L + (2 * f4) * PS + iy0 * 33 + ix0;
     v4f pre[8];
     auto commit = [&](int buf) {
@@ -449,7 +450,7 @@
         const v2f* p0 = lbase + buf * BUF + 132 * j;
         const v2f a = p0[0], c = p0[PS];
         v4f v; v[0] = a[0]; v[1] = a[1]; v[2] = c[0]; v[3] = c[1];
-        stg4(out + ob + tstr * j, v);
+        stg4(out + ob + tstro * j, v);
     };
     if (s_begin < s_end) {
         const long long b = pair_slice_base(g, s_begin) + toff;
@@ -462,7 +463,7 @@
         const int buf = (sl - s_begin) & 1;
         const bool more = sl + 1 < s_end, prev = sl > s_begin;
         const long long nb = pair_slice_base(g, more ? sl + 1 : sl) + toff;
-        const long long ob = pair_slice_base(g, prev ? sl - 1 : sl) + toff;
+        const long long ob = pair_slice_base(go, prev ? sl - 1 : sl) + toffo;
         v2f* P = L + buf * BUF + w * PS;
         v2f xc[4], xn[4];
 #pragma unroll
@@ -502,7 +503,7 @@
     }
     if (s_begin < s_end) {
         const int buf = (s_end - 1 - s_begin) & 1;
-        const long long ob = pair_slice_base(g, s_end - 1) + toff;
+        const long long ob = pair_slice_base(go, s_end - 1) + toffo;
 #pragma unroll
         for (int j = 0; j < 8; ++j) store1(buf, ob, j);
     }
@@ -510,6 +511,7 @@
 }
 static int pair_slices(const PairGeom& g) { return g.n0 * g.n1 * g.n2; }
 int plan_pair(PairItem* it, int n, int spw) {
+    for (int i = 0; i < n; ++i) if (it[i].go.n0 == 0) it[i].go = it[i].g;
     if (spw <= 0) {
         double tot = 0; for (int i = 0; i < n; ++i) tot += pair_slices(it[i].g); spw = 16; while (spw > 1 && 2.0 * tot / spw < 1024.0) spw >>= 1;
     }
@@ -531,7 +533,7 @@
     const int gw = blockIdx.x;
     const int lo = find_item(items, nitems, &PairGramItem::wg_begin, gw);
     const PairGramItem it = items[lo];
-    const PairGeom g = it.g;
+    const PairGeom g = it.g, gx = it.gx;
     const int nslices = g.n0 * g.n1 * g.n2;
     const int lw = gw - it.wg_begin;
     const int s_begin = lw * it.spw, s_end = min(nslices, s_begin + it.spw);
@@ -545,13 +547,12 @@
 #pragma unroll
     for (int r = 0; r < 16; ++r) { Or[r] = 0.f; Oi[r] = 0.f; }
     const int f = tid & 7, sg0 = tid >> 3;
-    const long long sx = g.sx, sy = g.sy, fo = (long long)f * g.cstr;
     v4f pre[16];
     const int ix0 = sg0 & 31, iy0 = sg0 >> 5;
-    const long long toff = fo + sx * ix0 + sy * iy0, tstr = 2 * sy;
     v2f* const lbase = L + (2 * f) * PS + iy0 * 33 + ix0;
-    auto issue = [&](const cf* __restrict__ G, int sl) {
-        const cf* p = G + pair_slice_base(g, sl) + toff;
+    auto issue = [&](const cf* __restrict__ G, const PairGeom& q, int sl) {
+        const cf* p = G + pair_slice_base(q, sl) + (long long)f * q.cstr + q.sx * ix0 + q.sy * iy0;
+        const long long tstr = 2 * q.sy;
 #pragma unroll
         for (int j = 0; j < 16; ++j) pre[j] = ldg4(p + tstr * j);
     };
@@ -564,12 +565,12 @@
         }
     };
 
-    if (s_begin < s_end) issue(Xg, s_begin);
+    if (s_begin < s_end) issue(Xg, gx, s_begin);
     for (int sl = s_begin; sl < s_end; ++sl) {
         lds_barrier();
         commit();
         lds_barrier();
-        issue(Yg, sl);
+        issue(Yg, g, sl);
         v16f C1r[2], C1i[2];
 #pragma unroll
         for (int pp = 0; pp < 2; ++pp) {
@@ -590,7 +591,7 @@
         lds_barrier();
         commit();
         lds_barrier();
-        if (sl + 1 < s_end) issue(Xg, sl + 1);
+        if (sl + 1 < s_end) issue(Xg, gx, sl + 1);
 #pragma unroll
         for (int pp = 0; pp < 2; ++pp) {
             const v2f* P = L + (w + 8 * pp) * PS;
@@ -625,6 +626,7 @@
     }
 }
 int plan_pair_gram(PairGramItem* it, int n, int* nwg, int spw) {
+    for (int i = 0; i < n; ++i) if (it[i].gx.n0 == 0) it[i].gx = it[i].g;
     if (spw <= 0) { double tot = 0; for (int i = 0; i < n; ++i) tot += pair_slices(it[i].g); spw = (int)std::max(4.0, std::min(16.0, tot / 2048.0)); }
     return lay_out(it, n, &PairGramItem::wg_begin, nwg, [&](PairGramItem& p) { p.spw = spw; return (pair_slices(p.g) + spw - 1) / spw; });
 }
@@ -645,7 +647,7 @@
     const int gw = blockIdx.x;
     const int lo = find_item(items, nitems, &PairGram2Item::wg_begin, gw);
     const PairGram2Item it = items[lo];
-    const PairGeom g = it.g;
+    const PairGeom g = it.g, gx = it.gx;
     const int nslices = g.n0 * g.n1 * g.n2;
     const int lw = gw - it.wg_begin;
     const int quarter = (lw >> 3) & 3, pw = ((lw >> 5) << 3) | (lw & 7);
@@ -664,6 +666,7 @@
     const int f2 = tid & 1, sg0 = tid >> 1;
     const int ix0 = sg0 & 31, iy0 = sg0 >> 5;
     const long long toff = (long long)(2 * quarter + f2) * g.cstr + g.sx * ix0 + g.sy * iy0, tstr = 8 * g.sy;
+    const long long toffx = (long long)(2 * quarter + f2) * gx.cstr + gx.sx * ix0 + gx.sy * iy0, tstrx = 8 * gx.sy;
     v2f* const lbase = L + (2 * f2) * PS + iy0 * 33 + ix0;
     v4f px[4], py[4];
     auto commit = [&](int buf) {
@@ -678,9 +681,9 @@
     };
     CAcc32<true> O; O.zero();
     if (s_begin < s_end) {
-        const long long b = pair_slice_base(g, s_begin) + toff;
-#pragma unroll
-        for (int j = 0; j < 4; ++j) { px[j] = ldg4(Xg + b + tstr * j); py[j] = ldg4(Yg + b + tstr * j); }
+        const long long b = pair_slice_base(g, s_begin) + toff, bx = pair_slice_base(gx, s_begin) + toffx;
+#pragma unroll
+        for (int j = 0; j < 4; ++j) { px[j] = ldg4(Xg + bx + tstrx * j); py[j] = ldg4(Yg + b + tstr * j); }
         commit(0);
     }
     lds_barrier();
@@ -691,6 +694,7 @@
         const bool more = sl + 1 < s_end;
         const v2f* PX = L + buf * BUF + comp * PS; const v2f* PY = PX + 4 * PS;
         const long long nb = pair_slice_base(g, more ? sl + 1 : sl) + toff;
+        const long long nbx = pair_slice_base(gx, more ? sl + 1 : sl) + toffx;
         auto xat = [&](int k) { return MSG ? PX[k * 33 + ln] : PX[ln * 33 + k]; };
         auto yat = [&](int k) { return MSG ? PY[k * 33 + ln] : PY[ln * 33 + k]; };
         v2f xc[4], xn[4];
@@ -712,7 +716,7 @@
                 else C.template mac_pre<false>(m0[q], mr[q], mi[q], xc[i][0], xc[i][1]);
                 if ((q & 1) == 0) {
                     const int j = q >> 2;
-                    if ((q & 2) == 0) px[j] = ldg4(Xg + nb + tstr * j); else py[j] = ldg4(Yg + nb + tstr * j);
+                    if ((q & 2) == 0) px[j] = ldg4(Xg + nbx + tstrx * j); else py[j] = ldg4(Yg + nb + tstr * j);
                     TNQS_PIN();
                 }
             }
@@ -761,6 +765,7 @@
 }
 int x3_pair_gram2_group();
 int plan_pair_gram2(PairGram2Item* it, int n, int* nwg, int spw) {
+    for (int i = 0; i < n; ++i) if (it[i].gx.n0 == 0) it[i].gx = it[i].g;
     auto groups = [](const PairGram2Item& p, int w) { const int np = (pair_slices(p.g) + w - 1) / w; return (np + 7) / 8; };
     if (spw <= 0)
         for (spw = 16; spw > 1; spw >>= 1) { long tot = 0; for (int i = 0; i < n; ++i) tot += 16 * groups(it[i], spw); if (tot >= 1024) break; }
diff --git a/tensornetworkquantumsimulator.jl_amd/csrc/kernels_x3.hip b/tensornetworkquantumsimulator.jl_amd/csrc/kernels_x3.hip
--- a/tensornetworkquantumsimulator.jl_amd/csrc/kernels_x3.hip
+++ b/tensornetworkquantumsimulator.jl_amd/csrc/kernels_x3.hip
@@ -22,7 +22,7 @@
     const int gw = blockIdx.x;
     const int lo = find_item(items, nitems, &PairGram2Item::wg_begin, gw);
     const PairGram2Item it = items[lo];
-    const PairGeom g = it.g;
+    const PairGeom g = it.g, gx = it.gx;
     const int nslices = g.n0 * g.n1 * g.n2;
     const int lw = gw - it.wg_begin;
     const int half = (lw >> 3) & 1, pw = ((lw >> 4) << 3) | (lw & 7);
@@ -44,6 +44,7 @@
     const int f4 = tid & 3, sg0 = tid >> 2;
     const int ix0 = sg0 & 31, iy0 = sg0 >> 5;
     const long long toff = (long long)(4 * half + f4) * g.cstr + g.sx * ix0 + g.sy * iy0, tstr = 4 * g.sy;
+    const long long toffx = (long long)(4 * half + f4) * gx.cstr + gx.sx * ix0 + gx.sy * iy0, tstrx = 4 * gx.sy;
     v2f* const lbase = L + (2 * f4) * PS + iy0 * P + ix0;
     v4f px[8], py[8];
     auto commit = [&]() {
@@ -60,9 +61,9 @@
 #pragma unroll
     for (int r = 0; r < 16; ++r) { Or[r] = 0.f; Oi[r] = 0.f; }
     if (s_begin < s_end) {
-        const long long b = x3_slice_base(g, s_begin) + toff;
-#pragma unroll
-        for (int j = 0; j < 8; ++j) { px[j] = ldg4(Xg + b + tstr * j); py[j] = ldg4(Yg + b + tstr * j); }
+        const long long b = x3_slice_base(g, s_begin) + toff, bx = x3_slice_base(gx, s_begin) + toffx;
+#pragma unroll
+        for (int j = 0; j < 8; ++j) { px[j] = ldg4(Xg + bx + tstrx * j); py[j] = ldg4(Yg + b + tstr * j); }
         commit();
     }
     lds_barrier();
@@ -82,6 +83,7 @@
     for (int sl = s_begin; sl < s_end; ++sl) {
         const bool more = sl + 1 < s_end;
         const long long nb = x3_slice_base(g, more ? sl + 1 : sl) + toff;
+        const long long nbx = x3_slice_base(gx, more ? sl + 1 : sl) + toffx;
         float ar[8], ai[8], br[8], bi[8];
         read8(L + comp * PS, 8 * h, 8 * h + 4, ar, ai);
 #pragma unroll
@@ -91,7 +93,7 @@
             read8(PX, 16 + 8 * h, 16 + 8 * h + 4, br, bi);
             if (t == 0) {
 #pragma unroll
-                for (int j = 0; j < 2; ++j) { px[j] = ldg4(Xg + nb + tstr * j); py[j] = ldg4(Yg + nb + tstr * j); }
+                for (int j = 0; j < 2; ++j) { px[j] = ldg4(Xg + nbx + tstrx * j); py[j] = ldg4(Yg + nb + tstr * j); }
             }
             TNQS_PIN();
             {
@@ -102,7 +104,7 @@
             read8(PY, 4 * h, 4 * h + 8, ar, ai);
             if (t == 0) {
 #pragma unroll
-                for (int j = 2; j < 4; ++j) { px[j] = ldg4(Xg + nb + tstr * j); py[j] = ldg4(Yg + nb + tstr * j); }
+                for (int j = 2; j < 4; ++j) { px[j] = ldg4(Xg + nbx + tstrx * j); py[j] = ldg4(Yg + nb + tstr * j); }
             }
             TNQS_PIN();
             {
@@ -113,7 +115,7 @@
             read8(PY, 16 + 4 * h, 16 + 4 * h + 8, br, bi);
             if (t == 0) {
 #pragma unroll
-                for (int j = 4; j < 6; ++j) { px[j] = ldg4(Xg + nb + tstr * j); py[j] = ldg4(Yg + nb + tstr * j); }
+                for (int j = 4; j < 6; ++j) { px[j] = ldg4(Xg + nbx + tstrx * j); py[j] = ldg4(Yg + nb + tstr * j); }
             }
             TNQS_PIN();
             {
@@ -126,7 +128,7 @@
             }
             if (t == 0) {
 #pragma unroll
-                for (int j = 6; j < 8; ++j) { px[j] = ldg4(Xg + nb + tstr * j); py[j] = ldg4(Yg + nb + tstr * j); }
+                for (int j = 6; j < 8; ++j) { px[j] = ldg4(Xg + nbx + tstrx * j); py[j] = ldg4(Yg + nb + tstr * j); }
             }
             if (t == 0 && !SINGLE) read8(L + (comp + 4) * PS, 8 * h, 8 * h + 4, ar, ai);
             TNQS_PIN();
@@ -178,6 +180,7 @@
 int x3_pair_gram2_group() { return 16; }
 int plan_x3_pair_gram1(PairGram2Item* it, int n, int* nwg, int spw) {
     auto slices = [](const PairGram2Item& p) { return p.g.n0 * p.g.n1 * p.g.n2; };
+    for (int i = 0; i < n; ++i) if (it[i].gx.n0 == 0) it[i].gx = it[i].g;
     if (spw <= 0) { double tot = 0; for (int i = 0; i < n; ++i) tot += (double)slices(it[i]); spw = 16; while (spw > 1 && 2.0 * tot / spw < 1024.0) spw >>= 1; }
     return lay_out(it, n, &PairGram2Item::wg_begin, nwg, [&](PairGram2Item& p) { p.spw = spw; const int np = (slices(p) + spw - 1) / spw; return 16 * ((np + 7) / 8); });
 }
@@ -206,7 +209,7 @@
     const int gw = blockIdx.x;
     const int lo = find_item(items, nitems, &PairItem::slice_begin, gw);
     const PairItem it = items[lo];
-    const PairGeom g = it.g;
+    const PairGeom g = it.g, go = it.go;
     const int nslices = g.n0 * g.n1 * g.n2;
     const int lw = gw - it.slice_begin;
     const int half = (lw >> 3) & 1, pw = ((lw >> 4) << 3) | (lw & 7);
@@ -232,6 +235,7 @@
     const int f4 = tid & 3, sg0 = tid >> 2;
     const int ix0 = sg0 & 31, iy0 = sg0 >> 5;
     const long long toff = (long long)(4 * half + f4) * g.cstr + g.sx * ix0 + g.sy * iy0, tstr = 4 * g.sy;
+    const long long toffo = (long long)(4 * half + f4) * go.cstr + go.sx * ix0 + go.sy * iy0, tstro = 4 * go.sy;
     v2f* const lbase = L + (2 * f4) * PS + iy0 * P + ix0;
     v4f preA[8], preB[8];
     #define TNQS_PIN() __builtin_amdgcn_sched_barrier(0x2 | 0x4)
@@ -247,7 +251,7 @@
         const v2f* p0 = lbase + buf * BUF + 4 * P * j;
         const v2f a = p0[0], c = p0[PS];
         v4f v; v[0] = a[0]; v[1] = a[1]; v[2] = c[0]; v[3] = c[1];
-        stg4(out + ob + tstr * j, v);
+        stg4(out + ob + tstro * j, v);
     };
     if (s_begin < s_end) {
         const long long b = x3_slice_base(g, s_begin) + toff;
@@ -262,7 +266,7 @@
     auto phase = [&](int sl, int buf, const v4f (&cur)[8], v4f (&nxt)[8]) {
         const bool more = sl + 1 < s_end, prev = sl > s_begin;
         const long long nb = x3_slice_base(g, sl + 2 < s_end ? sl + 2 : sl) + toff;
-        const long long ob = x3_slice_base(g, prev ? sl - 1 : sl) + toff;
+        const long long ob = x3_slice_base(go, prev ? sl - 1 : sl) + toffo;
         v2f* Pw = L + buf * BUF + w * PS;
         v16f Yr, Yi;
 #pragma unroll
@@ -307,7 +311,7 @@
     }
     if (s_begin < s_end) {
         const int buf = (s_end - 1 - s_begin) & 1;
-        const long long ob = x3_slice_base(g, s_end - 1) + toff;
+        const long long ob = x3_slice_base(go, s_end - 1) + toffo;
 #pragma unroll
         for (int j = 0; j < 8; ++j) store1(buf, ob, j);
     }
```

After: 6676. 1.5% lower.
